# cucibala/FaceRecognizeOnnx

Measured on AMD Instinct MI355X. Metric: faces/sec end-to-end (detect+align+embed), batch=128 640x640, higher is better.
Workload: dtype f32; 1 GPU; C-headline: 128 frames 640x640 per GPU, SCRFD det_500m + decode + NMS, first 1 face(s)/frame aligned to 112x112, IResNet-50 (w600k_r50) embed, L2-norm; frames_per_gpu=128, faces_per_frame=1, weights=synthetic seeded (det seed 100, rec seed 200), input_residency=HBM-resident before the timed region, gallery_rows=0, topk=0, parallelism=frame-sharded x1, no data-path collective

## Files before the change

### facerecognizeonnx_amd/_lib.py

```python
from __future__ import annotations

import ctypes as C
import os
import subprocess

import numpy as np

_HERE = os.path.dirname(os.path.abspath(__file__))
LIB_PATH = os.path.join(_HERE, "libfacehip.so")
CSRC = os.path.join(_HERE, "csrc")

FACE_DTYPE = np.dtype([("x", "<i4"), ("y", "<i4"), ("w", "<i4"), ("h", "<i4"),
                       ("score", "<f4"), ("lm", "<f4", (10,))])
assert FACE_DTYPE.itemsize == 60


class FhFace(C.Structure):
    _fields_ = [("x", C.c_int32), ("y", C.c_int32), ("w", C.c_int32), ("h", C.c_int32),
                ("score", C.c_float), ("lm", C.c_float * 10)]


class FhFrame(C.Structure):
    _fields_ = [("bgr", C.c_void_p), ("rows", C.c_int32), ("cols", C.c_int32), ("step", C.c_int32)]

# ... 111 lines not shown
    "fh_tracker_get_state": (_i, [_vp, _i, _vp, _ip, _ip]),
    "fh_track_plan": (_i, [_vp, _i, _i, _vp, _vp]),
    "fh_track_update_dev": (_i, [_vp, _vp, _vp, _i, _i, _vp, _vp, _vp, _vp]),
    "fh_track_select_dev": (_i, [_vp, _vp, _i, _i, _vp, _vp, _vp, _vp, _vp, _vp]),
    "fh_pipeline_run_tracked_dev": (_i, [_vp, _vp, _vp, _vp, _i, _i, _i, _i, _ll, _vp, _f, _f, _i, _vp, _vp, _vp, _vp, _vp, _vp, _vp, _vp]),
    "fh_track_update_slots_dev": (_i, [_vp, _vp, _vp, _i, _i, _vp, _vp, _vp, _vp, _vp]),
    "fh_tracker_enable_identity": (_i, [_vp, _i, _i]),
    "fh_track_identify_dev": (_i, [_vp, _vp, _f, _vp, _vp, _vp, _vp, _i, _i, _i, _vp, _vp, _vp, _vp]),
    "fh_tracker_queries_dev": (_vp, [_vp]),
    "fh_tracker_get_identity": (_i, [_vp, _i, _vp, _vp]),
    "fh_pipeline_run_identified_dev": (_i, [_vp, _vp, _vp, _vp, _f, _vp, _i, _i, _i, _i, _ll, _vp, _f, _f, _i, _vp, _vp, _vp, _vp, _vp, _vp, _vp,
                                            _vp, _vp, _vp]),
    "fh_face_quality_dev": (_i, [_vp, _i, _i, _i, _i, _ll, _vp, _vp, _i, _vp, _vp]),
    "fh_face_quality_ragged_dev": (_i, [_vp, _i, _vp, _vp, _i, _vp, _vp]),
    "fh_tracker_set_bestshot": (_i, [_vp, _i, _i, _i, _i]),
    "fh_tracker_get_quality": (_i, [_vp, _i, _vp]),
    "fh_tracker_quality_dev": (_vp, [_vp]),
    "fh_track_update_q_dev": (_i, [_vp, _vp, _vp, _i, _i, _vp, _vp, _vp, _vp, _vp, _vp]),
    "fh_track_identify_q_dev": (_i, [_vp, _vp, _f, _vp, _vp, _vp, _vp, _vp, _i, _i, _i, _vp, _vp, _vp, _vp]),
    "fh_tracker_enable_relink": (_i, [_vp, _i, _f, _i]),
    "fh_track_identify_link_dev": (_i, [_vp, _vp, _f, _vp, _vp, _vp, _vp, _vp, _i, _i, _i, _vp, _vp, _vp, _vp, _vp]),
    "fh_tracker_get_links": (_i, [_vp, _i, _vp, _vp]),
    "fh_tracker_roots_dev": (_vp, [_vp]),
    "fh_gallery_create": (_vp, [_i]),
    "fh_gallery_destroy": (None, [_vp]),
    "fh_gallery_upload": (_i, [_vp, _vp, _ll, _i, _ll]),
    "fh_gallery_enroll": (_ll, [_vp, _vp, _ll, _i]),
    "fh_gallery_size": (_ll, [_vp]),
    "fh_gallery_label_dev": (_i, [_vp, _vp, _i, _f, _vp, _vp, _vp]),
    "fh_gallery_topk_dev": (_i, [_vp, _vp, _i, _i, _vp, _vp, _vp]),
    "fh_gallery_set_scan": (_i, [_vp, _i]),
    "fh_gallery_get_scan": (_i, [_vp]),
    "fh_gallery_scan_stats": (_i, [_vp, C.POINTER(_ll), C.POINTER(_ll)]),
    "fh_topk_merge_dev": (_i, [_vp, _vp, _i, _i, _i, _vp, _vp, _vp]),
    "fh_gallery_enroll_ids": (_ll, [_vp, _vp, _vp, _ll, _i]),
    "fh_gallery_upload_ids": (_i, [_vp, _vp, _vp, _ll, _i, _ll]),
    "fh_gallery_topk_ids_dev": (_i, [_vp, _vp, _i, _i, _vp, _vp, _vp, _vp]),
    "fh_gallery_label_ids_dev": (_i, [_vp, _vp, _i, _f, _vp, _vp, _vp]),
    "fh_gallery_remove_ids": (_ll, [_vp, _vp, _ll]),
    "fh_gallery_get_ids": (_ll, [_vp, _ll, _ll, _vp]),
    "fh_topk_merge_ids_dev": (_i, [_vp, _vp, _vp, _i, _i, _i, _vp, _vp, _vp, _vp]),
    "fh_gallery_group_ids": (_ll, [_vp, _ll, _vp, _vp, _vp]),
    "fh_gallery_fuse_ids": (_ll, [_vp, _vp, _i]),
    "fh_gallery_get_rows": (_ll, [_vp, _ll, _ll, _vp]),
    "fh_gallery_self_scores_dev": (_i, [_vp, _vp, _vp, _vp]),
    "fh_cluster_scores": (_i, [_vp, _i, _f, _i, _i, _vp, _vp]),
    "fh_gallery_cluster_dev": (_i, [_vp, _f, _i, _i, _vp, _vp, _vp]),
    "fh_hist_bin": (_i, [_f]),
    "fh_roc_from_hist": (_i, [_vp, _d, _vp]),
    "fh_gallery_pair_hist_dev": (_i, [_vp, _vp, _vp, _vp]),
    "fh_gallery_set_ids": (_ll, [_vp, _vp, _i]),
    "fh_gallery_set_tags": (_ll, [_vp, _ll, _ll, _vp, _i]),
    "fh_gallery_get_tags": (_ll, [_vp, _ll, _ll, _vp]),
    "fh_gallery_topk_tagged_dev": (_i, [_vp, _vp, _vp, _i, _i, _vp, _vp, _vp]),
    "fh_gallery_topk_ids_tagged_dev": (_i, [_vp, _vp, _vp, _i, _i, _vp, _vp, _vp, _vp]),
    "fh_gallery_label_tagged_dev": (_i, [_vp, _vp, _vp, _i, _f, _vp, _vp, _vp]),
    "fh_gallery_label_ids_tagged_dev": (_i, [_vp, _vp, _vp, _i, _f, _vp, _vp, _vp]),
    "fh_gallery_tag_stats": (_i, [_vp, C.POINTER(_ll), C.POINTER(_ll)]),
    "fh_tracker_set_stream_masks": (_i, [_vp, _vp]),
    "fh_gallery_range_dev": (_i, [_vp, _vp, _vp, _i, _f, _i, _vp, _vp, _vp, _vp, _vp]),
    "fh_range_from_scores": (_i, [_vp, _ll, _ll, _vp, C.c_uint32, _f, _i, C.POINTER(_ll), _vp, _vp]),
    "fh_comm_unique_id": (_i, [_vp]),
    "fh_comm_create": (_vp, [_i, _i, _vp, _i]),
    "fh_comm_destroy": (None, [_vp]),
    "fh_comm_rank": (_i, [_vp]),
    "fh_comm_world": (_i, [_vp]),
    "fh_comm_allgather_f32_dev": (_i, [_vp, _vp, _vp, _ll, _vp]),
    "fh_gallery_topk_sharded_dev": (_i, [_vp, _vp, _vp, _i, _i, _vp, _vp, _vp]),
    "fh_timing_enable": (_i, [_i]),
    "fh_timing_num_tags": (_i, []),
    "fh_timing_collect": (_i, [_vp, _vp, _vp, _vp, _i]),
    "fh_timing_collect_ops": (_i, [_vp, _vp, _vp, _i]),
    "fh_det_set_conv_cfg": (_i, [_vp, _i, _i]),
    "fh_rec_set_conv_cfg": (_i, [_vp, _i, _i]),
    "fh_memcpy_d2h": (_i, [_vp, _vp, C.c_size_t]),
    "fh_det_sync": (_i, [_vp, _vp]),
    "fh_rec_sync": (_i, [_vp, _vp]),
    "fh_imread": (_i, [C.c_char_p, C.POINTER(_vp), C.POINTER(_i), C.POINTER(_i)]),
    "fh_image_decode": (_i, [_vp, C.c_size_t, C.POINTER(_vp), C.POINTER(_i), C.POINTER(_i)]),
    "fh_image_free": (None, [_vp]),
    "fh_det_set_winograd": (_i, [_vp, _i]),
    "fh_rec_set_winograd": (_i, [_vp, _i]),
    "fh_rec_set_wino_fusion": (_i, [_vp, _i]),
    "fh_rec_set_shortcut_fold": (_i, [_vp, _i]),
    "fh_rec_set_precision": (_i, [_vp, _i, C.POINTER(C.c_float)]),
    "fh_rec_get_precision": (_i, [_vp]),
    "fh_det_set_cus": (_i, [_vp, _i]),
    "fh_rec_set_cus": (_i, [_vp, _i]),
    "fh_debug_streamk": (_i, [_i, _i]),
    "fh_debug_wino_slots": (_i, [_i]),
    "fh_debug_cluster_tiles": (_i, [_i]),
    "fh_debug_hist_copies": (_i, [_i]),
    "fh_debug_tag_skip": (_i, [_i]),
    "fh_debug_topk_merge_strided_dev": (_i, [_vp, _vp, _i, _i, _i, _ll, _vp, _vp, _vp]),
    "fh_set_graph_replay": (_i, [_i]),
    "fh_det_workspace_dev": (_vp, [_vp]),
    "fh_det_graph_stats": (_i, [_vp, _vp]),
    "fh_rec_graph_stats": (_i, [_vp, _vp]),
    "fh_det_set_fused_stem": (_i, [_vp, _i]),
    "fh_rec_set_fused_stem": (_i, [_vp, _i]),
    "fh_det_set_fused_front": (_i, [_vp, _i]),
    "fh_det_set_halo_conv": (_i, [_vp, _i]),
    "fh_resize_u8c3_dev": (_i, [_vp, _i, _i, _i, _vp, _i, _i, _i, _vp]),
    "fh_conv_forward_dev": (_i, [_vp, _vp, _vp, _vp, _i, _i, _i, _i, _i, _i, _i, _i, _i, _vp]),
    "fh_conv_winograd_dev": (_i, [_vp, _vp, _vp, _vp, _i, _i, _i, _i, _i, _vp]),
    "fh_conv_winograd_ex_dev": (_i, [_vp, _vp, _vp, _vp, _i, _i, _i, _i, _i, _i, _vp]),
    "fh_debug_pack_bf16x2_dev": (_i, [_vp, _vp, _ll]),
    "fh_debug_wino_gemm_rows": (_ll, [_i, _i, _i, _i, _i, _i]),
    "fh_debug_wino_gemm_dev": (_i, [_vp, _vp, _vp, _i, _i, _i, _i, _i, _i, _i, _vp]),
    "fh_debug_wino2_clock_mhz": (_d, []),
    "fh_conv_wino2_dev": (_i, [_vp, _vp, _vp, _vp, _vp, _vp, _i, _i, _i, _i, _i, _i, _i, _vp]),
    "fh_conv_wino2_ex_dev": (_i, [_vp, _vp, _vp, _vp, _vp, _vp, _vp, _vp, _vp, _i, _vp, _vp, _vp, _i, _i, _i, _i, _i, _i, _i, _vp]),
    "fh_conv_wt_rows": (_i, [_i]),
    "fh_conv_pack_weights": (_i, [_vp, _i, _i, _i, _vp]),
    "fh_conv_kpad": (_i, [_i]),
}

_LIB = None


def lib() -> C.CDLL:
    global _LIB
    if _LIB is None:
        path = build()
        path = os.environ.get("FACEHIP_LIB") or path
        try:
            import torch
        except ImportError:
            pass
        L = C.CDLL(path)
        for name, (res, args) in PROTOTYPES.items():
            fn = getattr(L, name)
            fn.restype = res
            fn.argtypes = args
        _LIB = L
    return _LIB


def last_error() -> str:
    return lib().fh_last_error().decode(errors="replace")


class FaceHipError(RuntimeError):
    pass


def check(rc: int, what: str) -> int:
    if rc < 0:
        raise FaceHipError(f"{what} failed ({rc}): {last_error()}")
    return rc
```

### facerecognizeonnx_amd/api.py

```python
from __future__ import annotations

import ctypes as C
from dataclasses import dataclass, field
from typing import List, Optional

import numpy as np

from . import _lib
from ._lib import FACE_DTYPE, TRACK_DTYPE, check


@dataclass
class FaceBox:
    box: tuple = (0, 0, 0, 0)
    score: float = 0.0
    landmarks: np.ndarray = field(default_factory=lambda: np.zeros((5, 2), np.float32))

    def to_record(self) -> np.ndarray:
        r = np.zeros(1, FACE_DTYPE)
        r[0]["x"], r[0]["y"], r[0]["w"], r[0]["h"] = self.box
        r[0]["score"] = self.score
        r[0]["lm"] = np.asarray(self.landmarks, np.float32).reshape(10)
        return r

# ... 140 lines not shown
            return np.zeros(0, FACE_DTYPE)
        t = self.tiling() if tiling is None else _tiling(tiling)
        if max_faces is None:
            views = check(_lib.lib().fh_tile_plan(a.shape[0], a.shape[1], C.byref(t), None, 0), "fh_tile_plan")
            max_faces = max(1, self.num_anchors() * views)
        out = np.zeros(max_faces, FACE_DTYPE)
        n = check(_lib.lib().fh_det_detect_tiled(self._h, a.ctypes.data, a.shape[0], a.shape[1], a.strides[0], C.byref(t),
                                                  scoreThreshold, nmsThreshold, out.ctypes.data, max_faces), "fh_det_detect_tiled")
        return out[:n].copy()

    def sync(self, stream: int = 0) -> None:
        check(_lib.lib().fh_det_sync(self._h, stream), "fh_det_sync")


class FaceRecognizer:
    def __init__(self):
        self._h = None

    def __del__(self):
        self.close()

    def close(self):
        if getattr(self, "_h", None) and _lib is not None and getattr(_lib, "_LIB", None) is not None:
            _lib._LIB.fh_rec_destroy(self._h)
        self._h = None

    def loadModel(self, modelPath: str) -> bool:
        self.close()
        self._h = _lib.lib().fh_rec_create(str(modelPath).encode())
        return bool(self._h)

    def extractFeature(self, image, face) -> np.ndarray:
        if not self._h:
            return np.zeros(0, np.float32)
        a = _img(image)
        if a is None:
            return np.zeros(0, np.float32)
        rec = face.to_record() if isinstance(face, FaceBox) else np.asarray(face, FACE_DTYPE).reshape(1)
        dim = self.feature_dim()
        out = np.zeros(dim, np.float32)
        n = check(_lib.lib().fh_rec_extract(self._h, a.ctypes.data, a.shape[0], a.shape[1], a.strides[0],
                                             rec.ctypes.data, out.ctypes.data, dim), "fh_rec_extract")
        return out[:n]

    def extractFeatureSimple(self, image) -> np.ndarray:
        if not self._h:
            return np.zeros(0, np.float32)
        a = _img(image)
        if a is None:
            return np.zeros(0, np.float32)
        dim = self.feature_dim()
        out = np.zeros(dim, np.float32)
        n = check(_lib.lib().fh_rec_extract_simple(self._h, a.ctypes.data, a.shape[0], a.shape[1], a.strides[0],
                                                    out.ctypes.data, dim), "fh_rec_extract_simple")
        return out[:n]

    @staticmethod
    def compareFaces(feature1, feature2) -> float:
        f1 = np.ascontiguousarray(feature1, np.float32).reshape(-1)
        f2 = np.ascontiguousarray(feature2, np.float32).reshape(-1)
        return float(_lib.lib().fh_compare(f1.ctypes.data, f1.size, f2.ctypes.data, f2.size))

    @property
    def handle(self):
        return self._h

    def feature_dim(self) -> int:
        return _lib.lib().fh_rec_feature_dim(self._h)

    def macs_per_face(self) -> float:
        return _lib.lib().fh_rec_macs_per_face(self._h)

    def set_chunk(self, n: int):
        check(_lib.lib().fh_rec_set_chunk(self._h, n), "fh_rec_set_chunk")

    def set_precision(self, mode: str = "fp32") -> float:
        import ctypes as C
        modes = {"fp32": 0, "bf16x2": 1}
        if mode not in modes:
            raise ValueError(f"precision {mode!r}: expected one of {sorted(modes)}")
        worst = C.c_float(0.0)
        check(_lib.lib().fh_rec_set_precision(self._h, modes[mode], C.byref(worst)), "fh_rec_set_precision")
        return float(worst.value)

    def precision(self) -> str:
        return "bf16x2" if _lib.lib().fh_rec_get_precision(self._h) == 1 else "fp32"

    def embed_aligned_dev(self, crops_ptr: int, n: int, out_ptr: int, raw_ptr: int = 0, stream: int = 0) -> int:
        return check(_lib.lib().fh_rec_embed_aligned_dev(self._h, crops_ptr, n, out_ptr, raw_ptr, stream),
                     "fh_rec_embed_aligned_dev")

    def sync(self, stream: int = 0) -> None:
        check(_lib.lib().fh_rec_sync(self._h, stream), "fh_rec_sync")


def pipeline_run_dev(det: FaceDetector, rec: FaceRecognizer, frames_ptr: int, n: int, rows: int, cols: int,
                     faces_per_frame: int, faces_ptr: int, frame_of_ptr: int, emb_ptr: int,
                     scoreThreshold: float = 0.5, nmsThreshold: float = 0.4, stream: int = 0) -> int:
    step = cols * 3
    return check(_lib.lib().fh_pipeline_run_dev(det.handle, rec.handle, frames_ptr, n, rows, cols, step, rows * step,
                                                scoreThreshold, nmsThreshold, faces_per_frame, faces_ptr,
                                                frame_of_ptr, emb_ptr, stream), "fh_pipeline_run_dev")


def pipeline_run_ragged_dev(det: FaceDetector, rec: FaceRecognizer, frames, faces_per_frame: int, faces_ptr: int, frame_of_ptr: int,
                            emb_ptr: int, scoreThreshold: float = 0.5, nmsThreshold: float = 0.4, stream: int = 0) -> int:
    arr = frame_array(frames)
    return check(_lib.lib().fh_pipeline_run_ragged_dev(det.handle, rec.handle, arr, _frame_count(arr), scoreThreshold, nmsThreshold,
                                                       faces_per_frame, faces_ptr, frame_of_ptr, emb_ptr, stream),
                 "fh_pipeline_run_ragged_dev")


def pipeline_run_tiled_dev(det: FaceDetector, rec: FaceRecognizer, frames, tiling, faces_per_frame: int, faces_ptr: int,
                           frame_of_ptr: int, emb_ptr: int, scoreThreshold: float = 0.5, nmsThreshold: float = 0.4,
                           stream: int = 0) -> int:
    arr, t = frame_array(frames), _tiling(tiling)
    return check(_lib.lib().fh_pipeline_run_tiled_dev(det.handle, rec.handle, arr, _frame_count(arr), C.byref(t), scoreThreshold,
                                                      nmsThreshold, faces_per_frame, faces_ptr, frame_of_ptr, emb_ptr, stream),
                 "fh_pipeline_run_tiled_dev")


def _stream_of(stream_of, n: int):
    if stream_of is None:
        return None, None
    a = np.ascontiguousarray(np.asarray(stream_of, np.int32).reshape(-1))
    if a.size != n:
        raise ValueError(f"stream_of holds {a.size} entries for {n} frames")
    return a, a.ctypes.data


def track_plan(stream_of, streams: int):
    a = np.ascontiguousarray(np.asarray(stream_of, np.int32).reshape(-1))
    order, starts = np.empty(max(a.size, 1), np.int32), np.empty(max(int(streams), 0) + 1, np.int32)
    check(_lib.lib().fh_track_plan(a.ctypes.data if a.size else None, a.size, int(streams), order.ctypes.data, starts.ctypes.data),
          "fh_track_plan")
    return order[:a.size].copy(), starts


def face_quality_dev(frames, det_ptr: int, counts_ptr: int, per_frame: int, quality_ptr: int, n: Optional[int] = None,
                     rows: Optional[int] = None, cols: Optional[int] = None, step: Optional[int] = None, stream: int = 0) -> int:
    if n is None:
        arr = frame_array(frames)
        return check(_lib.lib().fh_face_quality_ragged_dev(arr, _frame_count(arr), det_ptr, counts_ptr, per_frame, quality_ptr, stream),
                     "fh_face_quality_ragged_dev")
    step = cols * 3 if step is None else step
    return check(_lib.lib().fh_face_quality_dev(frames, n, rows, cols, step, rows * step, det_ptr, counts_ptr, per_frame, quality_ptr,
                                                stream), "fh_face_quality_dev")


class Tracker:

    def __init__(self, streams: int = 1, max_tracks: int = _lib.TRACK_MAX, iou_thr: float = 0.3, max_missed: int = 0, refresh: int = 0):
        self._h = _lib.lib().fh_tracker_create(int(streams), int(max_tracks), float(iou_thr), int(max_missed), int(refresh))
        if not self._h:
            raise _lib.FaceHipError(f"fh_tracker_create failed: {_lib.last_error()}")
        self.streams, self.max_tracks = int(streams), int(max_tracks)

    def close(self):
        if getattr(self, "_h", None):
            _lib.lib().fh_tracker_destroy(self._h)
            self._h = None

    def __del__(self):
        self.close()

    @property
# ... 496 lines not shown
```

### facerecognizeonnx_amd/csrc/api.cpp

```cpp
#include <algorithm>
#include <cmath>
#include <cstddef>
#include <cstdio>
#include <cstring>
#include <memory>
#include <string>
#include <vector>

#include "../../include/facehip.h"
#include "cluster_plan.h"
#include "range_plan.h"
#include "roc_plan.h"
#include "engine.h"
#include "group_ids.h"
#include "track_plan.h"

static_assert(sizeof(fh_face) == 60 && sizeof(fh::FaceRec) == 60, "FaceBox mirror must stay 60 bytes");
static_assert(sizeof(fh_frame) == 24 && sizeof(fh::FrameIn) == 24 && offsetof(fh_frame, rows) == offsetof(fh::FrameIn, rows) &&
              offsetof(fh_frame, step) == offsetof(fh::FrameIn, step), "fh_frame and the engine's FrameIn are one layout");
static_assert(sizeof(fh_track_state) == sizeof(fh::TrackState) && offsetof(fh_track_state, hits) == offsetof(fh::TrackState, hits) &&
              FH_TRACK_MAX == 64, "fh_track_state mirrors TrackState; one slot per lane of a wave");
static_assert(sizeof(fh_track_ident) == 16 && sizeof(fh::TrackIdent) == 16 && offsetof(fh_track_ident, score) == offsetof(fh::TrackIdent, score),
              "fh_track_ident mirrors TrackIdent");
static_assert(sizeof(fh_track_link) == 32 && sizeof(fh::TrackLink) == 32 && offsetof(fh_track_link, last_seen) == offsetof(fh::TrackLink, last_seen) &&
// ... 1361 lines not shown
static_assert(FH_HIST_BINS == fh::kHistBins && sizeof(fh_roc_point) == sizeof(fh::RocPoint) && sizeof(unsigned long long) == sizeof(uint64_t) &&
              offsetof(fh_roc_point, bin) == offsetof(fh::RocPoint, bin) && offsetof(fh_roc_point, impostor) == offsetof(fh::RocPoint, impostor),
              "fh_roc_point mirrors roc_plan.h");
int fh_hist_bin(float score) { return fh::hist_bin(score); }
int fh_roc_from_hist(const unsigned long long* hist, double max_far, fh_roc_point out[2]) {
    if (!hist || !out) return arg_error("fh_roc_from_hist: null argument");
    if (!(max_far >= 0.0 && max_far <= 1.0)) return arg_error("fh_roc_from_hist: need 0 <= max_far <= 1");
    fh::RocPoint pt[2];
    if (fh::roc_from_hist(reinterpret_cast<const uint64_t*>(hist), max_far, pt) < 0) {
        g_err = "fh_roc_from_hist: a plane of the histogram is empty (no genuine or no impostor pairs)";
        return FH_ERR_STATE;
    }
    for (int k = 0; k < 2; ++k)
        out[k] = fh_roc_point{pt[k].threshold, pt[k].bin, pt[k].true_accepts, pt[k].false_accepts, pt[k].genuine, pt[k].impostor};
    return FH_OK;
}
int fh_gallery_pair_hist_dev(fh_gallery* g, unsigned long long* d_hist, unsigned long long* d_nan, void* stream) {
    if (!g || !d_hist) return arg_error("fh_gallery_pair_hist_dev: null argument");
    if (g->g.size() > 0 && !g->g.labelled()) {
        g_err = "gallery: fh_gallery_pair_hist_dev needs a labelled gallery (rows enrolled with ids, or fh_gallery_set_ids)";
        return FH_ERR_STATE;
    }
    return guarded([&] { g->g.pair_hist_dev(d_hist, d_nan, S(stream)); return (int)FH_OK; });
}
int fh_debug_hist_copies(int copies) { fh::cluster_debug_hist_copies(copies); return 0; }

static_assert(FH_RANGE_MAX_CAP == fh::kRangeMaxCap && FH_TAG_ALL == fh::kRangeTagAll, "facehip.h mirrors range_plan.h");
int fh_range_from_scores(const float* scores, long long n, long long index_base, const uint32_t* tags, uint32_t mask, float threshold, int cap,
                         long long* count, float* out_scores, int* out_indices) {
    int listed = -1;
    const int rc = guarded([&] {
        listed = fh::range_from_scores(scores, n, index_base, tags, mask, threshold, cap, count, out_scores, out_indices);
        return 0;
    });
    if (rc < 0) return rc;
    return listed < 0 ? arg_error("fh_range_from_scores: bad argument (null scores or count, NaN threshold, cap outside 1..1024, index beyond 31 bits)")
                      : listed;
}
int fh_gallery_range_dev(fh_gallery* g, const float* d_queries, const uint32_t* d_masks, int nq, float threshold, int cap, long long* d_counts,
                         float* d_scores, int* d_indices, int* d_ids, void* stream) {
    if (!g) return arg_error("fh_gallery_range_dev: null handle");
    if (nq < 0 || nq > 256) return arg_error("fh_gallery_range_dev: need 0 <= nq <= 256");
    if (cap < 1 || cap > FH_RANGE_MAX_CAP) return arg_error("fh_gallery_range_dev: need 1 <= cap <= FH_RANGE_MAX_CAP");
    if (threshold != threshold) return arg_error("fh_gallery_range_dev: the threshold is a NaN");
    if (g->g.dim() % 64) return arg_error("fh_gallery_range_dev: the gallery's dim must be a multiple of 64");
    if (nq == 0) return 0;
    if (!d_queries || !d_counts) return arg_error("fh_gallery_range_dev: null argument");
    if (d_ids && g->g.size() > 0 && !g->g.labelled()) {
        g_err = "gallery: fh_gallery_range_dev with d_ids needs a labelled gallery (rows enrolled with ids, or fh_gallery_set_ids)";
        return FH_ERR_STATE;
    }
    return guarded([&] { g->g.range_dev(d_queries, d_masks, nq, threshold, cap, d_counts, d_scores, d_indices, d_ids, S(stream)); return nq; });
}

int fh_debug_topk_merge_strided_dev(const float* ps, const int* pi, int nparts, int nq, int k, long long part_stride, float* scores, int* indices,
                                    void* stream) {
    if (!ps || !pi || !scores || !indices) return arg_error("fh_debug_topk_merge_strided_dev: null argument");
    if (nparts <= 0 || nq <= 0 || k <= 0 || k > 16 || (long)nparts * k > 65536 || part_stride < (long long)nq * k)
        return arg_error("fh_debug_topk_merge_strided_dev: bad size");
    return guarded([&] {
        fh::launch_topk_merge_strided(ps, pi, nparts, nq, k, (long)part_stride, scores, indices, S(stream));
        FH_HIP(hipGetLastError());
        return nq;
    });
}

int fh_timing_enable(int on) { fh::KernelTimer::get().enabled = on != 0; return FH_OK; }
int fh_timing_num_tags(void) { return fh::KernelTimer::kTags; }
int fh_timing_collect(double* ms, double* flops, double* bytes, long long* launches, int n) {
    if (!ms || !flops || !bytes || !launches || n < fh::KernelTimer::kTags) return arg_error("fh_timing_collect: need fh_timing_num_tags()-entry arrays");
    return guarded([&] { fh::KernelTimer::get().collect(ms, flops, bytes, launches); return fh::KernelTimer::kTags; });
}
int fh_timing_collect_ops(double* ms, double* flops, int* tag, int cap) {
    if (!ms || !flops || !tag || cap <= 0) return arg_error("fh_timing_collect_ops: bad argument");
    return guarded([&] { return fh::KernelTimer::get().collect_ops(ms, flops, tag, cap); });
}
int fh_det_set_conv_cfg(fh_det* d, int cfg, int stream_k) {
    if (!d) return arg_error("null handle");
    d->det.net().force_cfg = cfg; d->det.net().sk_enable = stream_k != 0;
    return FH_OK;
}
int fh_det_set_winograd(fh_det* d, int on) { if (!d) return arg_error("null handle"); d->det.net().winograd = on != 0; return FH_OK; }
int fh_rec_set_winograd(fh_rec* r, int on) { if (!r) return arg_error("null handle"); r->rec.net().winograd = on != 0; return FH_OK; }
int fh_rec_set_wino_fusion(fh_rec* r, int on) { if (!r) return arg_error("null handle"); r->rec.net().fuse_wino = on != 0; return FH_OK; }
int fh_rec_set_precision(fh_rec* r, int mode, float* worst_out) {
    if (!r || (mode != FH_PREC_FP32 && mode != FH_PREC_BF16X2)) return arg_error("fh_rec_set_precision: bad argument");
    if (worst_out) *worst_out = 0.f;
    Owns owns(&r->rec.net());
    if (mode == FH_PREC_FP32) return guarded([&] { r->rec.net().set_bf16x2(false, nullptr); return (int)FH_OK; });
    return guarded([&] {
        fh::Net& net = r->rec.net();
        const int n = 64, dim = r->rec.dim();
        const size_t crop = (size_t)net.in_h() * net.in_w() * 3;
        std::vector<uint8_t> h((size_t)n * crop);
        uint32_t st = 0x9E3779B9u;
        for (int i = 0; i < n; ++i) {
            const int amp = 16 + 3 * i;
            for (size_t e = 0; e < crop; ++e) {
                st = st * 1664525u + 1013904223u;
                const int px = (int)(e / 3) % net.in_w(), py = (int)(e / 3) / net.in_w();
                const int v = 128 + ((px * (i + 1) + py * (n - i)) % 97 - 48) + (int)((st >> 24) % (2 * amp + 1)) - amp;
                h[(size_t)i * crop + e] = (uint8_t)std::min(255, std::max(0, v));
            }
        }
        fh::DevBuf dc, de;
        dc.ensure(h.size()); de.ensure((size_t)2 * n * dim * sizeof(float));
        FH_HIP(hipMemcpy(dc.p, h.data(), h.size(), hipMemcpyHostToDevice));
        const bool was = net.bf16x2();
        net.set_bf16x2(false, nullptr);
        r->rec.embed_aligned_dev(dc.as<uint8_t>(), n, de.as<float>(), nullptr);
        const int layers = net.set_bf16x2(true, nullptr);
        if (layers == 0) { net.set_bf16x2(was, nullptr); throw std::runtime_error("fh_rec_set_precision: this model has no layer with a split-bf16 form"); }
        struct Rollback { fh::Net& n; bool armed = true; ~Rollback() { if (armed) { try { n.set_bf16x2(false, nullptr); } catch (...) {} } } } rollback{net};
        r->rec.embed_aligned_dev(dc.as<uint8_t>(), n, de.as<float>() + (size_t)n * dim, nullptr);
        std::vector<float> e((size_t)2 * n * dim);
        FH_HIP(hipDeviceSynchronize());
        FH_HIP(hipMemcpy(e.data(), de.p, e.size() * sizeof(float), hipMemcpyDeviceToHost));
        double worst = 0;
        for (int i = 0; i < n; ++i) {
            double dot = 0, na = 0, nb = 0;
            for (int c = 0; c < dim; ++c) {
                const double a = e[(size_t)i * dim + c], b = e[(size_t)(n + i) * dim + c];
                dot += a * b; na += a * a; nb += b * b;
            }
            const double err = (na > 0 && nb > 0) ? 1.0 - dot / std::sqrt(na * nb) : 1.0;
            worst = std::max(worst, std::isfinite(err) ? err : 1.0);
        }
        if (worst_out) *worst_out = (float)worst;
        double gate = 1e-3;
        if (const char* g = getenv("FACEHIP_PRECISION_GATE")) gate = std::min(gate, atof(g));
        if (!(worst < gate))
            throw std::runtime_error("fh_rec_set_precision: split-bf16 embeddings differ from fp32 by 1 - cos = " + std::to_string(worst) +
                                 " (gate " + std::to_string(gate) + "): staying fp32");
        rollback.armed = false;
        return layers;
    });
}
int fh_rec_get_precision(fh_rec* r) { return r && r->rec.net().bf16x2() ? FH_PREC_BF16X2 : FH_PREC_FP32; }
int fh_rec_set_shortcut_fold(fh_rec* r, int on) { if (!r) return arg_error("null handle"); r->rec.net().fold_shortcut = on != 0; return FH_OK; }
int fh_det_set_halo_conv(fh_det* d, int on) { if (!d) return arg_error("null handle"); d->det.net().halo_conv = on != 0; return FH_OK; }
int fh_det_set_cus(fh_det* d, int cus) { if (!d || cus < 0) return arg_error("bad argument"); d->det.net().cus = cus; return FH_OK; }
int fh_rec_set_cus(fh_rec* r, int cus) { if (!r || cus < 0) return arg_error("bad argument"); r->rec.net().cus = cus; return FH_OK; }
int fh_det_set_fused_stem(fh_det* d, int on) { if (!d) return arg_error("null handle"); d->det.net().fuse_stem = on != 0; return FH_OK; }
int fh_det_set_fused_front(fh_det* d, int on) { if (!d) return arg_error("null handle"); d->det.net().fuse_front = on != 0; return FH_OK; }
int fh_rec_set_fused_stem(fh_rec* r, int on) { if (!r) return arg_error("null handle"); r->rec.net().fuse_stem = on != 0; return FH_OK; }
int fh_rec_set_conv_cfg(fh_rec* r, int cfg, int stream_k) {
    if (!r) return arg_error("null handle");
    r->rec.net().force_cfg = cfg; r->rec.net().sk_enable = stream_k != 0;
    return FH_OK;
}

int fh_memcpy_d2h(void* dst, const void* src, size_t bytes) {
    if (!dst || !src) return arg_error("fh_memcpy_d2h: null argument");
    return guarded([&] { FH_HIP(hipDeviceSynchronize()); FH_HIP(hipMemcpy(dst, src, bytes, hipMemcpyDeviceToHost)); return 0; });
}
int fh_resize_u8c3_dev(const uint8_t* src, int sh, int sw, int sstep, uint8_t* dst, int dh, int dw, int dstep, void* stream) {
    if (!src || !dst || sh <= 0 || sw <= 0 || dh <= 0 || dw <= 0) return arg_error("fh_resize_u8c3_dev: bad argument");
    return guarded([&] {
        fh::launch_resize_u8c3(src, (long)sh * sstep, sh, sw, sstep, dst, (long)dh * dstep, dh, dw, dstep, 1, S(stream));
        FH_HIP(hipGetLastError());
        return 0;
    });
}
int fh_conv_winograd_ex_dev(const float* d_in, const float* w_ohwi, const float* d_bias, float* d_out, int batch, int h, int w, int cin,
                            int cout, int precision, void* stream) {
    if (!d_in || !w_ohwi || !d_out || cin % 32 || cout % 4 || (precision != FH_PREC_FP32 && precision != FH_PREC_BF16X2))
        return arg_error("fh_conv_winograd_dev: bad argument");
    const bool bf2 = precision == FH_PREC_BF16X2;
    Owns owns(nullptr);
    return guarded([&] {
        if (bf2 && !fh::wino_gemm_ok_bf16x2(cin, cout)) throw std::runtime_error("winograd: this layer has no split-bf16 GEMM");
        const int rows = fh::conv_wt_rows(cout);
        std::vector<float> u36((size_t)36 * rows * cin, 0.f), uf((size_t)cout * cin);
        std::vector<double> uall((size_t)cout * cin * 36);
        for (int co = 0; co < cout; ++co)
            for (int ci = 0; ci < cin; ++ci) {
                double g[9];
                for (int t = 0; t < 9; ++t) g[t] = w_ohwi[((size_t)co * 9 + t) * cin + ci];
                fh::wino_filter_transform(g, &uall[((size_t)co * cin + ci) * 36]);
            }
        for (int f = 0; f < 36; ++f) {
            for (size_t e = 0; e < uf.size(); ++e) uf[e] = (float)uall[e * 36 + f];
            fh::conv_pack_weights(uf.data(), cout, cin, 1, u36.data() + (size_t)f * rows * cin);
        }
        const size_t tiles = (size_t)batch * ((h + 3) / 4) * ((w + 3) / 4);
        fh::DevBuf dU, dV, dM;
        dU.ensure(u36.size() * sizeof(float));
        dV.ensure((36 * (size_t)fh::wino_rows((long)tiles) + 100 * 128) * cin * sizeof(float));
        dM.ensure((36 * (size_t)fh::wino_rows((long)tiles) + 100 * 128) * cout * sizeof(float));
        FH_HIP(hipMemcpy(dU.p, u36.data(), u36.size() * sizeof(float), hipMemcpyHostToDevice));
        fh::DevBuf dUp;
        if (bf2) {
            dUp.ensure(u36.size() * sizeof(float));
            fh::launch_pack_bf16x2(dU.as<float>(), dUp.as<float>(), (long)u36.size(), S(stream));
        }
        static fh::DevBuf slabs;
        static unsigned slabs_gen = 0;
        if (!slabs.p) { slabs.ensure(fh::conv_slab_floats() * sizeof(float)); fh::conv_workspace_init(slabs.as<float>()); slabs_gen = fh::conv_error_generation(); }
        if (slabs_gen != fh::conv_error_generation()) { fh::conv_workspace_reset_async(slabs.as<float>(), S(stream)); slabs_gen = fh::conv_error_generation(); }
        fh::ConvArgs a{};
        a.in = d_in; a.bias = d_bias; a.out1 = d_out; a.slabs = slabs.as<float>(); a.sk_enable = 1;
        a.B = batch; a.H = h; a.W = w; a.Ho = h; a.Wo = w; a.Cin = cin; a.Cout = cout; a.ks = 3; a.stride = 1; a.pad = 1;
        a.act = (int)fh::Act::NONE; a.res_mode = (int)fh::ResMode::NONE;
        fh::launch_conv_winograd(a, (bf2 ? dUp : dU).as<float>(), dV.as<float>(), dM.as<float>(), 2, nullptr, nullptr, S(stream), bf2);
        FH_HIP(hipStreamSynchronize(S(stream)));
        return 0;
    });
}
int fh_conv_winograd_dev(const float* d_in, const float* w_ohwi, const float* d_bias, float* d_out, int batch, int h, int w, int cin,
                         int cout, void* stream) {
    return fh_conv_winograd_ex_dev(d_in, w_ohwi, d_bias, d_out, batch, h, w, cin, cout, FH_PREC_FP32, stream);
}
int fh_debug_pack_bf16x2_dev(const float* d_in, float* d_out, long long n) {
    if (!d_in || !d_out || n < 0 || n % 4) return arg_error("fh_debug_pack_bf16x2_dev: bad argument (n % 4 == 0)");
    return guarded([&] {
        fh::launch_pack_bf16x2(d_in, d_out, (long)n, nullptr);
        FH_HIP(hipGetLastError());
        FH_HIP(hipStreamSynchronize(nullptr));
        return 0;
    });
}
static long long wino_gemm_rows(int batch, int h, int w, int k, int n, int mixed, fh::WinoPlanes* pl) {
    if (batch <= 0 || h <= 0 || w <= 0 || k <= 0 || n <= 0 || k % 32 || n % 32) return -1;
    if (!mixed) return 36LL * fh::wino_rows((long)batch * ((h + 3) / 4) * ((w + 3) / 4));
    fh::WinoPlanes p{};
    if (!fh::wino_mix_layout(batch, h, w, k, n, &p)) return -2;
    if (pl) *pl = p;
    return 128LL * p.total_tiles;
}
long long fh_debug_wino_gemm_rows(int batch, int h, int w, int k, int n, int mixed) {
    const long long r = wino_gemm_rows(batch, h, w, k, n, mixed, nullptr);
    if (r == -2) return arg_error("fh_debug_wino_gemm_rows: the mixed tiling does not apply to this layer");
    if (r < 0) return arg_error("fh_debug_wino_gemm_rows: bad argument (k % 32 == 0, n % 32 == 0)");
    return r;
}
int fh_debug_wino_gemm_dev(const float* d_V, const float* d_U, float* d_M, int batch, int h, int w, int k, int n, int precision, int mixed,
                           void* stream) {
    if (!d_V || !d_U || !d_M || (precision != FH_PREC_FP32 && precision != FH_PREC_BF16X2))
        return arg_error("fh_debug_wino_gemm_dev: bad argument");
    fh::WinoPlanes pl{};
    const long long rows = wino_gemm_rows(batch, h, w, k, n, mixed, &pl);
    if (rows == -2) return arg_error("fh_debug_wino_gemm_dev: the mixed tiling does not apply to this layer");
    if (rows < 0) return arg_error("fh_debug_wino_gemm_dev: bad argument (k % 32 == 0, n % 32 == 0)");
    const bool bf2 = precision == FH_PREC_BF16X2;
    Owns owns(nullptr);
    return guarded([&] {
        if (bf2 && !fh::wino_gemm_ok_bf16x2(k, n)) throw std::runtime_error("winograd: this layer has no split-bf16 GEMM");
        const size_t nv = (size_t)rows * k, nu = (size_t)36 * fh::conv_wt_rows(n) * k;
        fh::DevBuf dVp, dUp;
        if (bf2) {
            dVp.ensure(nv * sizeof(float)); dUp.ensure(nu * sizeof(float));
            fh::launch_pack_bf16x2(d_V, dVp.as<float>(), (long)nv, S(stream));
            fh::launch_pack_bf16x2(d_U, dUp.as<float>(), (long)nu, S(stream));
        }
        fh::ConvArgs a{};
        a.B = batch; a.H = h; a.W = w; a.Ho = h; a.Wo = w; a.Cin = k; a.Cout = n; a.ks = 3; a.stride = 1; a.pad = 1;
        a.act = (int)fh::Act::NONE; a.res_mode = (int)fh::ResMode::NONE;
        fh::launch_wino_gemm(a, bf2 ? dUp.as<float>() : d_U, bf2 ? dVp.as<float>() : d_V, d_M, 2, bf2, S(stream), mixed ? &pl : nullptr);
        FH_HIP(hipGetLastError());
        FH_HIP(hipStreamSynchronize(S(stream)));
        return 0;
    });
}
int fh_conv_wino2_ex_dev(const float* d_in, const float* w_ohwi, const float* d_bias, const float* d_slope, const float* d_res, float* d_out,
                         float* d_out2, const float* d_s2, const float* d_t2, int n_outs, float* const* d_outs, const int* oc0, const int* oact,
                         int batch, int h, int w, int cin, int cout, int act, int bias_cls, void* stream) {
    if (!d_in || !w_ohwi || batch <= 0 || h <= 0 || w <= 0 || cin != 64 || cout <= 0) return arg_error("fh_conv_wino2_dev: bad argument (cin = 64, positive sizes)");
    if (n_outs < 0 || n_outs > 3 || (n_outs > 0 && (!d_outs || !oc0 || !oact))) return arg_error("fh_conv_wino2_dev: bad merged-output description");
    if (n_outs == 0 && ((!d_out && !d_out2) || cout % 64)) return arg_error("fh_conv_wino2_dev: plain layers need an output and cout % 64 == 0");
    if (d_out2 && (!d_s2 || !d_t2)) return arg_error("fh_conv_wino2_dev: a second output needs its scale and shift");
    Owns owns(nullptr);
    return guarded([&] {
        fh::ConvArgs a{};
        a.in = d_in; a.bias = d_bias; a.slope = d_slope; a.res = d_res; a.out1 = d_out; a.out2 = d_out2; a.s2 = d_s2; a.t2 = d_t2;
        a.B = batch; a.H = h; a.W = w; a.Ho = h; a.Wo = w; a.Cin = cin; a.Cout = cout; a.ks = 3; a.stride = 1; a.pad = 1;
        a.act = act; a.bias_cls = bias_cls; a.res_mode = d_res ? (int)fh::ResMode::SAME : (int)fh::ResMode::NONE;
        a.n_outs = n_outs;
        for (int g = 0; g < n_outs; ++g) { a.outs[g] = d_outs[g]; a.oact[g] = oact[g]; a.oc0[g] = oc0[g]; }
        if (n_outs > 0) a.oc0[n_outs] = oc0[n_outs];
        if (!fh::wino2_ok(a)) throw std::runtime_error("fh_conv_wino2_dev: layer shape not supported by the fused F(2x2) kernel");
        std::vector<float> u(fh::wino2_weight_floats(cin, cout));
        fh::wino2_pack_weights(w_ohwi, cout, cin, u.data());
        fh::DevBuf dU;
        dU.ensure(u.size() * sizeof(float));
        FH_HIP(hipMemcpy(dU.p, u.data(), u.size() * sizeof(float), hipMemcpyHostToDevice));
        a.wt = dU.as<float>();
        fh::launch_wino2(a, S(stream));
        FH_HIP(hipGetLastError());
        FH_HIP(hipStreamSynchronize(S(stream)));
        return 0;
    });
}
int fh_conv_wino2_dev(const float* d_in, const float* w_ohwi, const float* d_bias, const float* d_slope, const float* d_res, float* d_out,
                      int batch, int h, int w, int cin, int cout, int act, int bias_cls, void* stream) {
    return fh_conv_wino2_ex_dev(d_in, w_ohwi, d_bias, d_slope, d_res, d_out, nullptr, nullptr, nullptr, 0, nullptr, nullptr, nullptr, batch, h, w,
                                cin, cout, act, bias_cls, stream);
}
double fh_debug_wino2_clock_mhz(void) { return fh::wino2_debug_clock_mhz(); }
int fh_conv_wt_rows(int cout) { return fh::conv_wt_rows(cout); }
int fh_conv_pack_weights(const float* w_ohwi, int cout, int cin, int ksize, float* dst_packed) {
    if (!w_ohwi || !dst_packed || cout <= 0 || cin <= 0) return arg_error("fh_conv_pack_weights: bad argument");
    memset(dst_packed, 0, (size_t)fh::conv_wt_rows(cout) * fh::conv_kpad(ksize * ksize * cin) * sizeof(float));
    fh::conv_pack_weights(w_ohwi, cout, cin, ksize, dst_packed);
    return 0;
}
int fh_conv_kpad(int ktot) { return fh::conv_kpad(ktot); }
const float* fh_det_workspace_dev(fh_det* d) { return d ? d->det.net().workspace() : nullptr; }
int fh_set_graph_replay(int on) { g_graph_replay = on != 0; return FH_OK; }
int fh_det_graph_stats(fh_det* d, long long* replays) {
    if (!d) return arg_error("null handle");
    if (replays) *replays = d->gcall.replays;
    return (int)d->gcall.nodes;
}
int fh_rec_graph_stats(fh_rec* r, long long* replays) {
    if (!r) return arg_error("null handle");
    if (replays) *replays = r->gcall.replays + r->gcall_simple.replays;
    return (int)(r->gcall.nodes ? r->gcall.nodes : r->gcall_simple.nodes);
}
int fh_debug_wino_slots(int slots) { fh::wino_debug_slots(slots); return 0; }
int fh_debug_streamk(int drop_publish, int timeout_ms) { fh::conv_debug_streamk(drop_publish, timeout_ms); return 0; }
int fh_conv_forward_dev(const float* in, const float* wt, const float* bias, float* out, int batch, int h, int w, int cin, int cout,
                        int ks, int stride, int kpad, int cfg, void* stream) {
    if (!in || !wt || !out || batch <= 0 || (ks != 1 && ks != 3) || cin % 4) return arg_error("fh_conv_forward_dev: bad argument");
    Owns owns(nullptr);
    return guarded([&] {
        fh::ConvArgs a{};
        const int pad = ks / 2;
        a.in = in; a.wt = wt; a.bias = bias; a.out1 = out;
        a.B = batch; a.H = h; a.W = w; a.Cin = cin; a.Cout = cout; a.ks = ks; a.stride = stride; a.pad = pad;
        a.Ho = (h + 2 * pad - ks) / stride + 1; a.Wo = (w + 2 * pad - ks) / stride + 1;
        a.Kpad = kpad;
        static fh::DevBuf slabs;
        static unsigned slabs_gen = 0;
        if (!slabs.p) { slabs.ensure(fh::conv_slab_floats() * sizeof(float)); fh::conv_workspace_init(slabs.as<float>()); slabs_gen = fh::conv_error_generation(); }
        if (slabs_gen != fh::conv_error_generation()) { fh::conv_workspace_reset_async(slabs.as<float>(), S(stream)); slabs_gen = fh::conv_error_generation(); }
        a.slabs = slabs.as<float>(); a.sk_enable = 1;
        fh::launch_conv(a, cfg, S(stream));
        FH_HIP(hipGetLastError());
        return 0;
    });
}
// ... 7 lines not shown
```

### facerecognizeonnx_amd/csrc/engine.cpp

```cpp
#include "engine.h"

#include "group_ids.h"
#include "roc_plan.h"
#include "track_plan.h"

#include <atomic>
#include <climits>
#include <cstdio>
#include <cstdlib>
#include <algorithm>
#include <cmath>
#include <cstring>

namespace fh {

void hip_check(hipError_t e, const char* what) {
    if (e != hipSuccess) throw std::runtime_error(std::string("HIP error: ") + hipGetErrorString(e) + " in " + what);
}

static std::atomic<unsigned long long> g_layout_epoch{1};
unsigned long long layout_epoch() { return g_layout_epoch.load(std::memory_order_relaxed); }

DevBuf::~DevBuf() {
    if (p) { (void)hipFree(p); g_layout_epoch.fetch_add(1, std::memory_order_relaxed); }
// ... 95 lines not shown
        for (int co = 0; co < c.Cout; ++co) {
            double tap_shift[9];
            for (int t = 0; t < 9; ++t) {
                double acc = 0;
                for (int ci = 0; ci < c.Cin; ++ci) acc += (double)c.weight[((size_t)co * 9 + t) * c.Cin + ci] * pr.t2[ci];
                tap_shift[t] = acc;
            }
            for (int ry = 0; ry < 3; ++ry)
                for (int rx = 0; rx < 3; ++rx) {
                    double b = c.bias[co];
                    for (int ky = 0; ky < 3; ++ky)
                        for (int kx = 0; kx < 3; ++kx) {
                            const bool in_y = !(ry == 0 && ky == 0) && !(ry == 2 && ky == 2);
                            const bool in_x = !(rx == 0 && kx == 0) && !(rx == 2 && kx == 2);
                            if (in_y && in_x) b += tap_shift[ky * 3 + kx];
                        }
                    b9[(size_t)(ry * 3 + rx) * c.Cout + co] = (float)b;
                }
            for (int t = 0; t < 9; ++t)
                for (int ci = 0; ci < c.Cin; ++ci) c.weight[((size_t)co * 9 + t) * c.Cin + ci] *= pr.s2[ci];
        }
        c.bias = b9;
        dev_[i].bn_fold_src = c.bn_src;
        dev_[c.bn_src].bn_fold_dst = true;
    }
    for (size_t i = 0; i < plan_.ops.size(); ++i) {
        const POp& op = plan_.ops[i];
        DevOp& d = dev_[i];
        if (op.kind == OpKind::DWPW) {
            d.dww = push(op.dw_weight.data(), op.dw_weight.size());
            d.dwb = push(op.dw_bias.data(), op.dw_bias.size());
        }
        if (op.kind == OpKind::CONV || op.kind == OpKind::GEMM || op.kind == OpKind::DWPW) {
            const int Ktot = op.ks * op.ks * op.Cin;
            d.Kpad = conv_kpad(Ktot);
            const int rows = conv_wt_rows(op.Cout);
            std::vector<float> packed((size_t)rows * d.Kpad, 0.f);
            conv_pack_weights(op.weight.data(), op.Cout, op.Cin, op.ks, packed.data());
            d.wt = push(packed.data(), packed.size());
            if (op.kind == OpKind::CONV) {
                ConvArgs probe{};
                probe.ks = op.ks; probe.stride = op.stride; probe.pad = op.pad; probe.Cin = op.Cin; probe.Cout = op.Cout; probe.act = (int)op.act;
                probe.res_mode = (int)op.res_mode; probe.H = op.H; probe.W = op.W;
                float dummy = 0.f;
                probe.out2 = op.out2 >= 0 ? &dummy : nullptr;
                probe.bias_cls = dev_[i].bn_fold_src >= 0 ? 1 : 0;
                if (conv_halo_ok(probe) && op.Ho * op.Wo >= 400) {
                    std::vector<float> wf(conv_halo_wfrag_floats(op.Cin, op.Cout));
                    conv_halo_pack_weights(op.weight.data(), op.Cout, op.Cin, wf.data());
                    d.wfrag = push(wf.data(), wf.size());
                    d.halo = true;
                }
            }
            if (op.kind == OpKind::CONV && op.Cin < kWinoMinCin) {
                ConvArgs probe{};
                probe.ks = op.ks; probe.stride = op.stride; probe.pad = op.pad; probe.Cin = op.Cin; probe.Cout = op.Cout; probe.act = (int)op.act;
                probe.res_mode = (int)op.res_mode; probe.H = op.H; probe.W = op.W; probe.Ho = op.Ho; probe.Wo = op.Wo;
                probe.n_outs = (int)op.outs.size(); probe.bias_cls = dev_[i].bn_fold_src >= 0 ? 1 : 0;
                float dummy2 = 0.f;
                probe.out2 = op.out2 >= 0 ? &dummy2 : nullptr;
                if (wino2_ok(probe)) {
                    std::vector<float> u(wino2_weight_floats(op.Cin, op.Cout));
                    wino2_pack_weights(op.weight.data(), op.Cout, op.Cin, u.data());
                    d.w2 = push(u.data(), u.size());
                    d.w2ok = true;
                }
            }
            if (op.kind == OpKind::CONV && op.ks == 3 && op.stride == 1 && op.pad == 1 && op.Cin >= kWinoMinCin && op.Cin % 32 == 0 &&
                op.Cout % 4 == 0 && op.outs.empty() && op.res_mode != ResMode::UP2X) {
                std::vector<float> u36((size_t)36 * rows * op.Cin, 0.f), uf((size_t)op.Cout * op.Cin);
                std::vector<double> uall((size_t)op.Cout * op.Cin * 36);
                for (int co = 0; co < op.Cout; ++co)
                    for (int ci = 0; ci < op.Cin; ++ci) {
                        double g[9];
                        for (int t = 0; t < 9; ++t) g[t] = op.weight[((size_t)co * 9 + t) * op.Cin + ci];
                        wino_filter_transform(g, &uall[((size_t)co * op.Cin + ci) * 36]);
                    }
                for (int f = 0; f < 36; ++f) {
                    for (size_t e = 0; e < uf.size(); ++e) uf[e] = (float)uall[e * 36 + f];
                    conv_pack_weights(uf.data(), op.Cout, op.Cin, 1, u36.data() + (size_t)f * rows * op.Cin);
                }
                d.w36 = push(u36.data(), u36.size());
                d.w36n = u36.size();
                d.wino = true;
                d.bf2 = wino_gemm_ok_bf16x2(op.Cin, op.Cout);
                const size_t tiles = (size_t)((op.H + 3) / 4) * ((op.W + 3) / 4);
                wino_elems_ = std::max(wino_elems_, 36 * tiles * (size_t)std::max(op.Cin, op.Cout));
                wino_maxc_ = std::max(wino_maxc_, (size_t)std::max(op.Cin, op.Cout));
            }
        } else if (op.kind == OpKind::DWCONV || op.kind == OpKind::DWGLOBAL || op.kind == OpKind::GCONV) {
            d.wt = push(op.weight.data(), op.weight.size());
        }
        if (!op.bias.empty()) d.bias = push(op.bias.data(), op.bias.size());
        if (!op.slope.empty()) { d.slope = push(op.slope.data(), op.slope.size()); d.has_slope = true; }
        if (!op.s2.empty()) { d.s2 = push(op.s2.data(), op.s2.size()); d.t2 = push(op.t2.data(), op.t2.size()); d.has_aff = true; }
    }
    for (size_t i = 0; i < plan_.ops.size(); ++i) {
        const POp& c = plan_.ops[i];
        if (c.sc_src < 0 || dev_[i].bn_fold_src >= 0 || c.bias.size() != (size_t)c.Cout) continue;
        if (dev_[i].wino || dev_[i].halo) continue;
        const POp& x = plan_.ops[c.sc_src];
        const int K9 = 9 * c.Cin, K = K9 + x.Cin, rows = conv_wt_rows(c.Cout);
        std::vector<float> w((size_t)rows * K, 0.f), b((size_t)c.Cout);
        for (int co = 0; co < c.Cout; ++co) {
            std::copy_n(&c.weight[(size_t)co * K9], K9, &w[(size_t)co * K]);
            std::copy_n(&x.weight[(size_t)co * x.Cin], x.Cin, &w[(size_t)co * K + K9]);
            b[co] = c.bias[co] + (x.bias.empty() ? 0.f : x.bias[co]);
        }
        dev_[i].wt_sc = push(w.data(), w.size());
        dev_[i].bias_sc = push(b.data(), b.size());
        dev_[i].Kpad_sc = K;
        dev_[i].sc_src = c.sc_src;
        dev_[c.sc_src].sc_dst = true;
    }
    for (size_t i = 0; i < plan_.ops.size(); ++i) {
        const int prod = plan_.ops[i].bn_src;
        if (!dev_[i].wino || prod <= 0 || !dev_[prod].has_aff) continue;
        dev_[i].aff_src = prod; dev_[prod].aff_dst = (int)i;
    }
    for (size_t i = 0; i + 1 < plan_.ops.size(); ++i) {
        const POp& a = plan_.ops[i];
        const POp& b = plan_.ops[i + 1];
        if (!dev_[i].wino || !dev_[i + 1].wino || a.H != b.H || a.W != b.W || a.Cout != b.Cin || !wino_can_fuse(a.H, a.W, a.Cout, false)) continue;
        int feed = -1;
        if (dev_[i + 1].aff_src == (int)i) feed = 1;
        else if (a.out >= 0 && b.in == a.out) feed = 0;
        else if (a.out2 >= 0 && b.in == a.out2) feed = 1;
        if (feed < 0) continue;
        int other_uses = 0;
        if (a.out >= 0) {
            for (const POp& o : plan_.ops)
                for (int x : {o.in, o.in2, o.res}) if (x == a.out) ++other_uses;
            for (const auto& o : plan_.outputs) if (o.tensor == a.out) ++other_uses;
            if (b.in == a.out) --other_uses;
        }
        const bool writes_out2 = a.out2 >= 0 && dev_[i + 1].aff_src != (int)i;
        if (!wino_can_fuse(a.H, a.W, a.Cout, other_uses > 0 || a.res >= 0 || writes_out2)) continue;
        dev_[i].fuse_next = true; dev_[i].fuse_feed_aff = feed == 1; dev_[i].fuse_keep_out1 = other_uses > 0;
    }
    {
        const POp& op = plan_.ops[0];
        stem_ok_ = op.kind == OpKind::CONV && op.in == plan_.input && op.ks == 3 && op.Cin == 4 && op.res < 0 && op.outs.empty() &&
                   op.Cout % 4 == 0 && op.Cout <= 64 && (op.stride == 1 || op.stride == 2);
        if (stem_ok_) {
            std::vector<float> w27((size_t)27 * op.Cout);
            for (int co = 0; co < op.Cout; ++co)
                for (int t = 0; t < 9; ++t)
                    for (int ci = 0; ci < 3; ++ci) w27[(size_t)(t * 3 + ci) * op.Cout + co] = op.weight[((size_t)co * 9 + t) * 4 + ci];
            dev_[0].w27 = push(w27.data(), w27.size());
            std::vector<float> wf((size_t)27 * op.Cout), bf((size_t)op.Cout);
            for (int co = 0; co < op.Cout; ++co) {
                double sum = 0;
                for (int t = 0; t < 9; ++t)
                    for (int j = 0; j < 3; ++j) {
                        const float w = op.weight[((size_t)co * 9 + t) * 4 + (2 - j)];
                        wf[(size_t)(t * 3 + j) * op.Cout + co] = w / 128.0f;
                        sum += w;
                    }
                bf[co] = (float)((double)op.bias[co] - 127.5 / 128.0 * sum);
            }
            dev_[0].wf = push(wf.data(), wf.size());
            dev_[0].bf = push(bf.data(), bf.size());
            if (op.Cout % 16 == 0) {
                std::vector<unsigned> fr((size_t)(op.Cout / 16) * 3 * 64 * 4, 0u);
                stem_pack_wfrag(wf.data(), op.Cout, fr.data());
                std::vector<float> asf(fr.size());
// ... 24 lines not shown
    (void)hipDeviceSynchronize();
    if (device >= 0 && device != cur && cur >= 0) (void)hipSetDevice(cur);
    conv_error_record_release(p);
}

void Net::reserve(int max_batch) {
    if (max_batch <= cap_) return;
    cap_ = max_batch;
    arena_.ensure(plan_.arena_elems * (size_t)cap_ * sizeof(float));
    if (partial_.bytes < conv_slab_floats() * sizeof(float)) {
        partial_.ensure(conv_slab_floats() * sizeof(float));
        conv_workspace_init(partial_.as<float>());
        if (!sk_rec_.p) { sk_rec_.p = conv_error_record_new(); (void)hipGetDevice(&sk_rec_.device); }
        if (!sk_rec_.p) throw std::runtime_error("HIP error: cannot allocate the stream-K watchdog record");
        sk_gen_ = conv_error_generation();
    }
    if (wino_elems_) {
        const size_t pad = 36 * 256 * wino_maxc_;
        wino_v_.ensure((wino_elems_ * (size_t)cap_ + pad) * sizeof(float));
        wino_m_.ensure((wino_elems_ * (size_t)cap_ + pad) * sizeof(float));
    }
    FH_HIP(hipMemset(arena_.p, 0, arena_.bytes));
}

void Net::run_u8(const uint8_t* src, long img_stride, int srcH, int srcW, int step, int batch, hipStream_t s) {
    if (batch <= 0) return;
    if (batch > cap_) throw std::runtime_error("Net::run_u8: batch exceeds reserved capacity");
    if (stem_ok_ && fuse_stem && front_ok_ && fuse_front && srcW >= 2) {
        const POp& st = plan_.ops[0];
        const POp& op = plan_.ops[1];
        const DevOp& d0 = dev_[0];
        const DevOp& d = dev_[1];
        const float* P = params_.as<float>();
        ConvArgs a{};
        a.wt = P + d.wt; a.bias = P + d.bias;
        a.out1 = tensor_ptr(op.out);
        a.dw_w = P + d.dww; a.dw_b = P + d.dwb; a.dw_act = (int)op.dw_act; a.dw_stride = op.dw_stride;
        a.B = batch; a.H = op.H; a.W = op.W; a.Cin = op.Cin; a.Ho = op.Ho; a.Wo = op.Wo; a.Cout = op.Cout;
        a.ks = 1; a.stride = 1; a.pad = 0; a.Kpad = d.Kpad; a.act = (int)op.act;
        a.u8_src = src; a.u8_img_stride = img_stride; a.u8_step = step; a.u8_srcH = srcH; a.u8_srcW = srcW; a.u8_inH = plan_.inH; a.u8_inW = plan_.inW;
        a.slabs = partial_.as<float>();
        a.u8_stride = st.stride; a.stem_act = (int)st.act; a.stem_wf = P + d0.wf; a.stem_bf = P + d0.bf;
        a.stem_wfrag = reinterpret_cast<const unsigned*>(P + d0.wfr);
        a.cus = cus;
        a.t_flops = 2.0 * (st.macs + op.macs) * batch;
        a.t_bytes = ((double)srcH * srcW * 3 + (double)op.Ho * op.Wo * op.Cout * 4) * batch;
        launch_dwpw(a, s);
        run(batch, s, 2);
        return;
    }
    if (stem_ok_ && fuse_stem) {
        const POp& op = plan_.ops[0];
        const DevOp& d = dev_[0];
        const float* P = params_.as<float>();
        KernelTimer& timer = KernelTimer::get();
        timer.begin(s);
        StemArgs a{};
        a.src = src; a.img_stride = img_stride; a.srcH = srcH; a.srcW = srcW; a.step = step; a.B = batch; a.inH = plan_.inH; a.inW = plan_.inW;
        a.stride = op.stride; a.Cout = op.Cout; a.w27 = P + d.w27; a.bias = P + d.bias; a.wf = P + d.wf; a.biasf = P + d.bf;
        a.wfrag = d.wfr ? reinterpret_cast<const unsigned*>(P + d.wfr) : nullptr;
        a.slope = d.has_slope ? P + d.slope : nullptr; a.act = (int)op.act; a.cus = cus;
        a.out1 = op.out >= 0 ? tensor_ptr(op.out) : nullptr; a.out2 = op.out2 >= 0 && !d.bn_fold_dst ? tensor_ptr(op.out2) : nullptr;
        if (d.has_aff) { a.s2 = P + d.s2; a.t2 = P + d.t2; }
        launch_stem(a, s);
        timer.end(s, 5, 2.0 * op.macs * batch, op.bytes * batch);
        run(batch, s, 1);
        return;
    }
    launch_det_preprocess(src, img_stride, srcH, srcW, step, batch, plan_.inH, plan_.inW, srcH, srcW, input(), s);
    run(batch, s, 0);
}

int Net::set_bf16x2(bool on, hipStream_t s) {
    int layers = 0;
    size_t total = 0;
    for (auto& d : dev_) if (d.wino && d.bf2) { d.w36p = total; total += d.w36n; ++layers; }
    if (on && layers > 0 && w36_bf_.bytes < total * sizeof(float)) {
        w36_bf_.ensure(total * sizeof(float));
        for (const auto& d : dev_)
            if (d.wino && d.bf2) launch_pack_bf16x2(params_.as<float>() + d.w36, w36_bf_.as<float>() + d.w36p, (long)d.w36n, s);
        FH_HIP(hipStreamSynchronize(s));
    }
    bf16x2_ = on && layers > 0;
    return on ? layers : 0;
}

void Net::run(int batch, hipStream_t s, int first_op) {
    if (batch <= 0) return;
    if ((sk_gen_ != conv_error_generation() || conv_error_pending(sk_rec_.p)) && partial_.p) {
        conv_workspace_reset_async(partial_.as<float>(), s);
        sk_gen_ = conv_error_generation();
    }
    if (batch > cap_) throw std::runtime_error("Net::run: batch exceeds reserved capacity");
    const float* P = params_.as<float>();
    KernelTimer& timer = KernelTimer::get();
    bool v_ready = false;
    for (size_t i = (size_t)first_op; i < plan_.ops.size(); ++i) {
        const POp& op = plan_.ops[i];
        const DevOp& d = dev_[i];
        int tag = 5;
        const bool dense = op.kind == OpKind::CONV || op.kind == OpKind::GEMM || op.kind == OpKind::DWPW;
        if (!dense) timer.begin(s);
        switch (op.kind) {
            case OpKind::CONV:
            case OpKind::GEMM: {
                if (d.sc_dst && fold_shortcut && force_cfg < 0) break;
                ConvArgs a{};
                a.in = tensor_ptr(op.in);
                a.wt = P + d.wt;
                a.bias = P + d.bias;
                a.slope = d.has_slope ? P + d.slope : nullptr;
                a.res = op.res >= 0 ? tensor_ptr(op.res) : nullptr;
                a.out1 = op.out >= 0 ? tensor_ptr(op.out) : nullptr;
                a.out2 = op.out2 >= 0 ? tensor_ptr(op.out2) : nullptr;
                if (d.bn_fold_dst) a.out2 = nullptr;
                if (d.bn_fold_src >= 0) { a.in = tensor_ptr(plan_.ops[d.bn_fold_src].out); a.bias_cls = 1; }
                if (d.aff_dst >= 0 && winograd) {
                    const POp& c = plan_.ops[d.aff_dst];
                    if ((long)batch * ((c.H + 3) / 4) * ((c.W + 3) / 4) >= kWinoMinTiles) a.out2 = nullptr;
                }
                a.s2 = d.has_aff ? P + d.s2 : nullptr;
                a.t2 = d.has_aff ? P + d.t2 : nullptr;
                a.slabs = partial_.as<float>();
                a.sk_err = sk_rec_.p;
                a.sk_enable = sk_enable ? 1 : 0;
                a.cus = cus;
                a.no_pw = force_cfg >= 0 ? 1 : 0;
                a.B = batch; a.H = op.H; a.W = op.W; a.Cin = op.Cin; a.Ho = op.Ho; a.Wo = op.Wo; a.Cout = op.Cout;
                a.ks = op.ks; a.stride = op.stride; a.pad = op.pad; a.Kpad = d.Kpad;
                a.act = (int)op.act; a.res_mode = (int)op.res_mode;
                a.n_outs = (int)op.outs.size();
                for (int g = 0; g < a.n_outs && g < 3; ++g) { a.outs[g] = tensor_ptr(op.outs[g]); a.oact[g] = op.out_act[g]; a.oc0[g] = op.out_c0[g]; }
                if (a.n_outs > 0) a.oc0[a.n_outs] = op.out_c0[a.n_outs];
                const long M = (long)batch * op.Ho * op.Wo;
                int cfg = force_cfg >= 0 ? force_cfg : conv_pick_cfg(M, op.Cout);
                if (force_cfg < 0 && cfg == 0 && ((M + 127) / 128) * ((op.Cout + 127) / 128) < 128) cfg = 3;
                a.t_flops = 2.0 * op.macs * batch; a.t_bytes = op.bytes * batch;
                if (d.sc_src >= 0 && fold_shortcut && force_cfg < 0) {
                    const POp& x = plan_.ops[d.sc_src];
                    a.wt = P + d.wt_sc; a.bias = P + d.bias_sc; a.Kpad = d.Kpad_sc;
                    a.res = nullptr; a.res_mode = (int)ResMode::NONE;
                    a.sc_in = tensor_ptr(x.in); a.sc_H = x.H; a.sc_W = x.W; a.sc_C = x.Cin; a.sc_stride = x.stride;
                    a.t_flops += 2.0 * x.macs * batch;
                }
                if (d.halo && halo_conv && force_cfg < 0) {
                    launch_conv_halo(a, P + d.wfrag, s);
                    tag = 9;
                    break;
                }
                if (d.w2ok && winograd && force_cfg < 0 && d.sc_src < 0 && wino2_blocks(a) >= wino2_min_blocks()) {
                    a.wt = P + d.w2;
                    launch_wino2(a, s);
                    break;
                }
                const bool use_wino = d.wino && winograd && (long)batch * ((op.H + 3) / 4) * ((op.W + 3) / 4) >= kWinoMinTiles;
                if (use_wino) {
                    const int wcfg = force_cfg >= 0 ? force_cfg : 2;
                    const bool bf2 = bf16x2_ && d.bf2 && force_cfg < 0;
                    WinoPlanes pl;
                    const bool mix = wcfg == 2 && wino_mix_layout(batch, op.H, op.W, op.Cin, op.Cout, &pl);
                    if (!v_ready) {
                        const float* in_s = nullptr; const float* in_t = nullptr;
                        if (d.aff_src >= 0) {
                            a.in = tensor_ptr(plan_.ops[d.aff_src].out);
                            in_s = P + dev_[d.aff_src].s2; in_t = P + dev_[d.aff_src].t2;
                        }
                        if (mix) launch_wino_mix(a, pl, nullptr, wino_v_.as<float>(), 0, in_s, in_t, bf2, s);
                        else launch_wino_input(a, wino_v_.as<float>(), in_s, in_t, bf2, s);
                    }
                    launch_wino_gemm(a, bf2 ? w36_bf_.as<float>() + d.w36p : P + d.w36, wino_v_.as<float>(), wino_m_.as<float>(), wcfg, bf2, s,
                                     mix ? &pl : nullptr);
                    v_ready = false;
                    if (d.fuse_next && fuse_wino && i + 1 < plan_.ops.size()) {
                        const POp& nx = plan_.ops[i + 1];
                        const bool next_wino = dev_[i + 1].wino && (long)batch * ((nx.H + 3) / 4) * ((nx.W + 3) / 4) >= kWinoMinTiles;
                        const bool next_mix = next_wino && wcfg == 2 && wino_mix_layout(batch, nx.H, nx.W, nx.Cin, nx.Cout, nullptr);
                        if (next_wino && mix == next_mix) {
                            ConvArgs e = a;
                            if (!d.fuse_keep_out1) e.out1 = nullptr;
                            const bool pack_next = bf16x2_ && dev_[i + 1].bf2 && force_cfg < 0;
                            if (mix) launch_wino_mix(e, pl, wino_m_.as<float>(), wino_v_.as<float>(), d.fuse_feed_aff ? 1 : 0, nullptr, nullptr, pack_next, s);
                            else launch_wino_fused(e, wino_m_.as<float>(), wino_v_.as<float>(), d.fuse_feed_aff ? 1 : 0, pack_next, s);
                            v_ready = true;
                        }
                    }
                    if (!v_ready) {
                        if (mix) launch_wino_mix(a, pl, wino_m_.as<float>(), nullptr, 0, nullptr, nullptr, false, s);
                        else launch_wino_output(a, wino_m_.as<float>(), s);
                    }
                    tag = 7;
                    break;
                }
                launch_conv(a, cfg, s);
                tag = cfg;
                break;
            }
            case OpKind::DWPW: {
                ConvArgs a{};
                a.in = tensor_ptr(op.in);
                a.wt = P + d.wt; a.bias = P + d.bias;
                a.out1 = tensor_ptr(op.out);
                a.dw_w = P + d.dww; a.dw_b = P + d.dwb; a.dw_act = (int)op.dw_act; a.dw_stride = op.dw_stride;
                a.B = batch; a.H = op.H; a.W = op.W; a.Cin = op.Cin; a.Ho = op.Ho; a.Wo = op.Wo; a.Cout = op.Cout;
                a.ks = 1; a.stride = 1; a.pad = 0; a.Kpad = d.Kpad; a.act = (int)op.act;
                a.t_flops = 2.0 * op.macs * batch; a.t_bytes = op.bytes * batch;
                a.slabs = partial_.as<float>();
                a.cus = cus;
                launch_dwpw(a, s);
                break;
            }
            case OpKind::DWCONV:
                launch_dwconv3x3(tensor_ptr(op.in), P + d.wt, P + d.bias, tensor_ptr(op.out), batch, op.H, op.W, op.Cin, op.stride,
                                 (int)op.act, d.has_slope ? P + d.slope : nullptr, s);
                tag = 4;
                break;
            case OpKind::DWGLOBAL:
                launch_dwglobal(tensor_ptr(op.in), P + d.wt, P + d.bias, tensor_ptr(op.out), batch, op.ks * op.ks, op.Cin, (int)op.act,
                                d.has_slope ? P + d.slope : nullptr, s);
                break;
            case OpKind::GCONV:
                launch_gconv3x3(tensor_ptr(op.in), P + d.wt, P + d.bias, tensor_ptr(op.out), batch, op.H, op.W, op.Cin,
                                (int)(op.weight_group), op.stride, (int)op.act, d.has_slope ? P + d.slope : nullptr, s);
                tag = 4;
                break;
            case OpKind::AFFINE:
                launch_affine(tensor_ptr(op.in), P + d.s2, P + d.t2, tensor_ptr(op.out), (long)batch * op.H * op.W, op.Cin, s);
                break;
            case OpKind::ACT:
                launch_act(tensor_ptr(op.in), d.has_slope ? P + d.slope : nullptr, tensor_ptr(op.out), (long)batch * op.H * op.W,
                           op.Cin, (int)op.act, s);
                break;
            case OpKind::ADD:
                launch_add(tensor_ptr(op.in), tensor_ptr(op.in2), tensor_ptr(op.out), (long)batch * op.H * op.W * op.Cin, s);
                break;
            case OpKind::UPSAMPLE:
                launch_upsample2x(tensor_ptr(op.in), tensor_ptr(op.out), batch, op.H, op.W, op.Cin, s);
                break;
        }
        if (!dense) timer.end(s, tag, 2.0 * op.macs * batch, op.bytes * batch);
        if (debug_sync()) {
            fprintf(stderr, "[facehip] op %zu %s batch %d done-launch\n", i, op.name.c_str(), batch); fflush(stderr);
            const hipError_t e1 = hipGetLastError(), e2 = hipStreamSynchronize(s);
            if (e1 != hipSuccess || e2 != hipSuccess)
                throw std::runtime_error("HIP error after op " + std::to_string(i) + " (" + op.name + "): " + hipGetErrorString(e1 != hipSuccess ? e1 : e2));
        }
    }
    FH_HIP(hipGetLastError());
}

Detector::Detector(const std::string& onnx_path) : net_(onnx_path, 640, 640) {
    const auto& outs = net_.plan().outputs;
    const int H = net_.in_h(), W = net_.in_w();
    if (outs.size() == 9) {
        static const int cols[9] = {1, 1, 1, 4, 4, 4, 10, 10, 10};
// ... 173 lines not shown
}

void TileTable::upload(const TilePlan& p, hipStream_t s) {
    const size_t vb = p.views.size() * sizeof(ViewDesc), sb = p.segs.size() * sizeof(FrameSeg);
    char* h = static_cast<char*>(st_.stage(vb + sb));
    if (vb) memcpy(h, p.views.data(), vb);
    if (sb) memcpy(h + vb, p.segs.data(), sb);
    V_ = (int)p.views.size();
    st_.send(vb + sb, s);
}

void postprocess_views(PostArgs a, int n_frames, const TileTable* tab, float nms_thr, int* sup, FaceRec* out, int max_out, int* counts,
                       hipStream_t s) {
    FH_HIP(hipMemsetAsync(a.count, 0, (size_t)n_frames * sizeof(int), s));
    a.views = tab ? tab->views() : nullptr;
    a.segs = tab ? tab->segs() : nullptr;
    if (a.rows) launch_rows_threshold(a, s);
    else launch_scrfd_decode(a, s);
    launch_sort_nms(a.cand, a.keys, a.count, a.segs, a.cap, n_frames, nms_thr, out, counts, max_out, sup, s);
    FH_HIP(hipGetLastError());
}

PostArgs Detector::post_source(int V, float score_thr) {
    PostArgs a{};
    if (predecoded_) { a.rows = net_.output(0); a.n_rows = anchors_; a.feat = feat_; }
    else {
        for (int i = 0; i < 3; ++i) { a.score[i] = net_.output(i); a.bbox[i] = net_.output(3 + i); a.kps[i] = net_.output(6 + i); }
        a.inH = net_.in_h(); a.inW = net_.in_w();
    }
    a.V = V; a.cap = cap_; a.border = -1; a.thr = score_thr;
    a.cand = cand_.as<FaceRec>(); a.keys = keys_.as<unsigned long long>(); a.count = count_.as<int>();
    return a;
}

int Detector::run_network_tiled_dev(const FrameIn* frames, int n, const Tiling& t, hipStream_t s) {
    const int V = tplan_.plan(frames, n, t, net_.in_w(), net_.in_h(), cap_, kTileMaxViews);
    if (V < 0) throw std::invalid_argument("tiled detection: more than FH_TILE_MAX_VIEWS views in one call, split the batch");
    frames_table_.upload(frames, n, 0, 0, s);
    ttab_.upload(tplan_, s);
    if (V > 0) run_network_ragged_dev(tplan_.view_frames.data(), V, s);
    return V;
}

void Detector::detect_tiled_dev(const FrameIn* frames, int n, const Tiling& t, float score_thr, float nms_thr, FaceRec* out, int max_out,
                                int* counts, hipStream_t s) {
    if (n <= 0) return;
    const int V = run_network_tiled_dev(frames, n, t, s);
    if (V == 0 || anchors_ <= 0) { FH_HIP(hipMemsetAsync(counts, 0, (size_t)n * sizeof(int), s)); return; }
    keys_.ensure(tplan_.key_total * sizeof(unsigned long long));
    ws_.ensure(tplan_.key_total * sizeof(int));
    count_.ensure((size_t)n * sizeof(int));
    PostArgs a = post_source(V, score_thr);
    a.border = t.border;
    postprocess_views(a, n, &ttab_, nms_thr, ws_.as<int>(), out, max_out, counts, s);
}

void Detector::run_input_dev(const float* input, int n, hipStream_t s) {
    reserve(n, 0, 0);
    ragged_ = false;
    const size_t per = (size_t)net_.in_h() * net_.in_w() * 4;
    FH_HIP(hipMemcpyAsync(net_.input(), input, (size_t)n * per * sizeof(float), hipMemcpyDeviceToDevice, s));
    net_.run(n, s);
}

void Detector::postprocess_dev(int n, float score_thr, float nms_thr, FaceRec* out, int max_out, int* counts, hipStream_t s) {
    if (anchors_ <= 0) { FH_HIP(hipMemsetAsync(counts, 0, (size_t)n * sizeof(int), s)); return; }
    if (ragged_ && n > table_.size()) throw std::runtime_error("detector: more frames than the last ragged call described");
    PostArgs a = post_source(n, score_thr);
    a.scale = scale_;
    a.scales = ragged_ ? table_.scales() : nullptr;
    postprocess_views(a, n, nullptr, nms_thr, ws_.as<int>(), out, max_out, counts, s);
}

void Detector::detect_dev(const uint8_t* frames, int n, int rows, int cols, int step, long stride, float score_thr, float nms_thr,
                          FaceRec* out, int max_out, int* counts, hipStream_t s) {
    if (n <= 0) return;
    run_network_dev(frames, n, rows, cols, step, stride, s);
    postprocess_dev(n, score_thr, nms_thr, out, max_out, counts, s);
}

Recognizer::Recognizer(const std::string& onnx_path) : net_(onnx_path, 112, 112) {
    const auto& o = net_.plan().outputs.at(0);
    dim_ = o.rows * o.cols;
}

void Recognizer::embed_aligned_dev(const uint8_t* crops, int n, float* out, hipStream_t s, float* raw_out) {
    const int H = net_.in_h(), W = net_.in_w();
    net_.reserve(std::min(n, max_chunk));
    for (int off = 0; off < n; off += max_chunk) {
        const int c = std::min(max_chunk, n - off);
        net_.run_u8(crops + (size_t)off * H * W * 3, (long)H * W * 3, H, W, W * 3, c, s);
        if (raw_out) FH_HIP(hipMemcpyAsync(raw_out + (size_t)off * dim_, net_.output(0), (size_t)c * dim_ * sizeof(float), hipMemcpyDeviceToDevice, s));
        launch_l2_normalize(net_.output(0), out + (size_t)off * dim_, c, dim_, s);
    }
    FH_HIP(hipGetLastError());
}

void Recognizer::embed_input_dev(const float* input, int n, float* out, hipStream_t s, float* raw_out) {
    const size_t per = (size_t)net_.in_h() * net_.in_w() * 4;
    net_.reserve(std::min(n, max_chunk));
    for (int off = 0; off < n; off += max_chunk) {
        const int c = std::min(max_chunk, n - off);
        FH_HIP(hipMemcpyAsync(net_.input(), input + (size_t)off * per, (size_t)c * per * sizeof(float), hipMemcpyDeviceToDevice, s));
        net_.run(c, s);
        if (raw_out) FH_HIP(hipMemcpyAsync(raw_out + (size_t)off * dim_, net_.output(0), (size_t)c * dim_ * sizeof(float), hipMemcpyDeviceToDevice, s));
        launch_l2_normalize(net_.output(0), out + (size_t)off * dim_, c, dim_, s);
    }
    FH_HIP(hipGetLastError());
}

void Recognizer::align_dev(const uint8_t* frames, int rows, int cols, int step, long stride, const FaceRec* faces,
                           const int* frame_of, int n, uint8_t* crops, int* ok, hipStream_t s) {
    launch_align(frames, stride, rows, cols, step, faces, frame_of, n, net_.in_h(), net_.in_w(), crops, ok, s);
    FH_HIP(hipGetLastError());
}

void Recognizer::embed_faces_dev(const uint8_t* frames, int rows, int cols, int step, long stride, const FaceRec* faces,
                                 const int* frame_of, int n, float* out, int* ok, hipStream_t s) {
    if (n <= 0) return;
    const size_t crop = (size_t)net_.in_h() * net_.in_w() * 3;
    crops_.ensure((size_t)n * crop);
    ok_.ensure((size_t)n * sizeof(int));
    int* okp = ok ? ok : ok_.as<int>();
    align_dev(frames, rows, cols, step, stride, faces, frame_of, n, crops_.as<uint8_t>(), okp, s);
    embed_aligned_dev(crops_.as<uint8_t>(), n, out, s);
}

void Recognizer::align_table_dev(const FrameDesc* table, int n_frames, const FaceRec* faces, const int* frame_of, int n, uint8_t* crops,
                                 int* ok, hipStream_t s) {
    launch_align_ragged(table, n_frames, faces, frame_of, n, net_.in_h(), net_.in_w(), crops, ok, s);
    FH_HIP(hipGetLastError());
}

void Recognizer::embed_faces_table_dev(const FrameDesc* table, int n_frames, const FaceRec* faces, const int* frame_of, int n, float* out,
                                       int* ok, hipStream_t s) {
    if (n <= 0) return;
    const size_t crop = (size_t)net_.in_h() * net_.in_w() * 3;
    crops_.ensure((size_t)n * crop);
    ok_.ensure((size_t)n * sizeof(int));
    align_table_dev(table, n_frames, faces, frame_of, n, crops_.as<uint8_t>(), ok ? ok : ok_.as<int>(), s);
    embed_aligned_dev(crops_.as<uint8_t>(), n, out, s);
}

void Recognizer::align_ragged_dev(const FrameIn* frames, int n_frames, const FaceRec* faces, const int* frame_of, int n, uint8_t* crops,
                                  int* ok, hipStream_t s) {
    align_table_dev(table_.upload(frames, n_frames, 0, 0, s), n_frames, faces, frame_of, n, crops, ok, s);
}

void Recognizer::embed_faces_ragged_dev(const FrameIn* frames, int n_frames, const FaceRec* faces, const int* frame_of, int n, float* out,
                                        int* ok, hipStream_t s) {
    if (n <= 0) return;
    embed_faces_table_dev(table_.upload(frames, n_frames, 0, 0, s), n_frames, faces, frame_of, n, out, ok, s);
}

void Recognizer::resize_embed_dev(const uint8_t* frames, int n, int rows, int cols, int step, long stride, float* out, hipStream_t s) {
    const int H = net_.in_h(), W = net_.in_w();
    crops_.ensure((size_t)n * H * W * 3);
    launch_resize_u8c3(frames, stride, rows, cols, step, crops_.as<uint8_t>(), (long)H * W * 3, H, W, W * 3, n, s);
    embed_aligned_dev(crops_.as<uint8_t>(), n, out, s);
}

Tracker::Tracker(int streams, int max_tracks, float iou_thr, int max_missed, int refresh)
    : streams_(streams), p_{max_tracks, iou_thr, max_missed, refresh, 1, 1, 1} {
    state_.ensure((size_t)streams * (2 * sizeof(int) + (size_t)max_tracks * sizeof(TrackState)));
    reset(-1);
}
// ... 189 lines not shown
```

### facerecognizeonnx_amd/csrc/engine.h

```cpp
#pragma once
#include <hip/hip_runtime.h>

#include <cstdint>
#include <stdexcept>
#include <string>
#include <utility>
#include <vector>

#include "kernels.h"
#include "plan.h"
#include "tile_plan.h"

namespace fh {


struct DevBuf {
    void* p = nullptr;
    size_t bytes = 0;
    DevBuf() = default;
    DevBuf(const DevBuf&) = delete;
    DevBuf& operator=(const DevBuf&) = delete;
    ~DevBuf();
    void ensure(size_t n);
    void swap(DevBuf& o) { std::swap(p, o.p); std::swap(bytes, o.bytes); }
    void grow(size_t n, size_t keep) {
        if (n <= bytes) return;
        if (keep == 0) return ensure(n);
        DevBuf bigger;
        bigger.ensure(n);
        FH_HIP(hipMemcpy(bigger.p, p, keep, hipMemcpyDeviceToDevice));
        swap(bigger);
    }
    template <class T> T* as() const { return reinterpret_cast<T*>(p); }
};

unsigned long long layout_epoch();

class Net {
  public:
    Net(const std::string& onnx_path, int default_h, int default_w);
    void reserve(int max_batch);
    float* input() const { return arena_.as<float>() + plan_.tensors[plan_.input].offset * (size_t)cap_; }
    float* output(int i) const { return tensor_ptr(plan_.outputs[i].tensor); }
    void run(int batch, hipStream_t s, int first_op = 0);
    void run_u8(const uint8_t* src, long img_stride, int srcH, int srcW, int step, int batch, hipStream_t s);
    bool fuse_stem = true;
    bool fuse_front = true;
    const Plan& plan() const { return plan_; }
    int in_h() const { return plan_.inH; }
    int in_w() const { return plan_.inW; }
    int capacity() const { return cap_; }
    bool winograd = true;
    bool halo_conv = true;
    bool fold_shortcut = true;
    bool fuse_wino = true;
    int set_bf16x2(bool on, hipStream_t s);
    bool bf16x2() const { return bf16x2_; }
    int cus = 0;
    int force_cfg = -1;
    bool sk_enable = true;
    long long config_word() const {
        return (long long)fuse_stem | (long long)fuse_front << 1 | (long long)winograd << 2 | (long long)halo_conv << 3 |
               (long long)fold_shortcut << 4 | (long long)fuse_wino << 5 | (long long)bf16x2_ << 6 | (long long)sk_enable << 7 |
               (long long)(cus & 0xffff) << 8 | (long long)((force_cfg + 1) & 0xff) << 24;
    }

  private:
    struct DevOp {
        size_t wt = 0, bias = 0, slope = 0, s2 = 0, t2 = 0;
        bool has_slope = false, has_aff = false;
        size_t w27 = 0;
        size_t wfr = 0;
        size_t wf = 0, bf = 0;
        size_t dww = 0, dwb = 0;
        size_t w36 = 0;
        size_t w36n = 0, w36p = 0;
        bool bf2 = false;
        size_t wfrag = 0;
        bool halo = false;
        bool wino = false;
        size_t w2 = 0;
        bool w2ok = false;
        int aff_src = -1;
        int aff_dst = -1;
        int bn_fold_src = -1;
        bool bn_fold_dst = false;
        int sc_src = -1;
        size_t wt_sc = 0, bias_sc = 0;
        int Kpad_sc = 0;
        bool sc_dst = false;
        bool fuse_next = false;
        bool fuse_feed_aff = false;
        bool fuse_keep_out1 = true;
        int Kpad = 0;
    };
  public:
    float* workspace() const { return partial_.as<float>(); }
    unsigned* error_record() const { return sk_rec_.p; }
  private:
    float* tensor_ptr(int t) const { return arena_.as<float>() + plan_.tensors[t].offset * (size_t)cap_; }
    Plan plan_;
    std::vector<DevOp> dev_;
    DevBuf params_, arena_, partial_, wino_v_, wino_m_, w36_bf_;
    bool bf16x2_ = false;
    size_t wino_maxc_ = 0;
    size_t wino_elems_ = 0;
    int cap_ = 0;
    struct SkRecord {
        unsigned* p = nullptr;
        int device = -1;
        SkRecord() = default;
        SkRecord(const SkRecord&) = delete;
        SkRecord& operator=(const SkRecord&) = delete;
        ~SkRecord();
    } sk_rec_;
    unsigned sk_gen_ = 0;
    bool stem_ok_ = false;
    bool front_ok_ = false;
};

int letterbox_plan(int rows, int cols, int in_w, int in_h, int* new_w, int* new_h, float* scale);

struct FrameIn {
    const uint8_t* bgr;
    int32_t rows, cols, step;
};
inline bool frame_empty(const FrameIn& f) { return !f.bgr || f.rows <= 0 || f.cols <= 0; }

class StagedTable {
  public:
    StagedTable() = default;
    StagedTable(const StagedTable&) = delete;
    StagedTable& operator=(const StagedTable&) = delete;
    ~StagedTable();
    void* stage(size_t bytes);
    void* send(size_t bytes, hipStream_t s);
    void* dev() const { return dev_.p; }

  private:
    static constexpr int kSlots = 4;
    struct Slot { void* p = nullptr; size_t bytes = 0; hipEvent_t ev = nullptr; bool pending = false; } slot_[kSlots];
    int next_ = 0, cur_ = 0;
    DevBuf dev_;
};

class FrameTable {
  public:
    const FrameDesc* upload(const FrameIn* frames, int n, int in_w, int in_h, hipStream_t s);
    const FrameDesc* table() const { return static_cast<const FrameDesc*>(st_.dev()); }
    const float* scales() const { return reinterpret_cast<const float*>(table() + n_); }
    int size() const { return n_; }

  private:
    int n_ = 0;
    StagedTable st_;
};

struct TilePlan {
    std::vector<FrameIn> view_frames;
    std::vector<ViewDesc> views;
    std::vector<FrameSeg> segs;
    size_t key_total = 0;
    int plan(const FrameIn* frames, int n, const Tiling& t, int in_w, int in_h, int cap, int max_views);
};
constexpr int kTileMaxViews = 256;

class TileTable {
  public:
    void upload(const TilePlan& p, hipStream_t s);
    const ViewDesc* views() const { return static_cast<const ViewDesc*>(st_.dev()); }
    const FrameSeg* segs() const { return reinterpret_cast<const FrameSeg*>(views() + V_); }

  private:
    int V_ = 0;
    StagedTable st_;
};

void postprocess_views(PostArgs a, int n_frames, const TileTable* tab, float nms_thr, int* sup, FaceRec* out, int max_out, int* counts,
                       hipStream_t s);

class Detector {
  public:
    explicit Detector(const std::string& onnx_path);
    void detect_dev(const uint8_t* frames, int n, int rows, int cols, int step, long stride, float score_thr, float nms_thr,
                    FaceRec* out, int max_out, int* counts, hipStream_t s);
    Net& net() { return net_; }
    int num_anchors() const { return anchors_; }
// ... 180 lines not shown
```

### facerecognizeonnx_amd/csrc/gemm_tile.h

```cpp
#pragma once
#include <hip/hip_runtime.h>

#include "kernels.h"

namespace fh {

typedef float v4f __attribute__((ext_vector_type(4)));
typedef float v16f __attribute__((ext_vector_type(16)));
typedef unsigned v4u __attribute__((ext_vector_type(4)));
typedef __bf16 bf16x8 __attribute__((ext_vector_type(8)));

__device__ __forceinline__ void lds_dma16(const float* src, void* dst) {
#if defined(__HIP_DEVICE_COMPILE__)
    __builtin_amdgcn_global_load_lds(src, (__attribute__((address_space(3))) void*)dst, 16, 0, 0);
#else
    (void)src; (void)dst;
#endif
}

template <typename I>
__device__ __forceinline__ int xcd_tile(const I block, const int nblocks) {
    const int q = nblocks >> 3, r8 = nblocks & 7, x = block & 7;
    return x * q + min(x, r8) + (int)(block >> 3);
}
// ... 31 lines not shown
}

template <int BN>
__device__ __forceinline__ void gemm_load_chunk(GemmSrc& s, const int buf, const bool a_live = true, const float* const a_dead = nullptr) {
    v4f* const dA = s.dA + buf * gemm_buf_slots<BN>();
    v4f* const dB = s.dB + buf * gemm_buf_slots<BN>();
#pragma unroll
    for (int i = 0; i < GEMM_BM / 32; ++i) lds_dma16(a_live ? s.a + i * s.a32 : a_dead, dA + i * 32 * 8);
#pragma unroll
    for (int i = 0; i < BN / 32; ++i) lds_dma16(s.b + i * s.b32, dB + i * 32 * 8);
    s.a += 32; s.b += 32;
}

template <int TN>
struct GemmFrag {
    v4f x, w[TN];
};
template <int TN>
__device__ __forceinline__ GemmFrag<TN> gemm_frag(const v4f* const tile, const GemmLane& l, const int s) {
    const v4f* const X = tile + l.wid * (32 * 8) + l.fr * 8;
    const v4f* const Wt = tile + GEMM_BM * 8 + l.fr * 8;
    const int col = (2 * s + l.fh2) ^ l.fsw;
    GemmFrag<TN> f;
    f.x = X[col];
#pragma unroll
    for (int j = 0; j < TN; ++j) f.w[j] = Wt[j * 32 * 8 + col];
    return f;
}

template <int BN, int ABL = 0>
__device__ __forceinline__ void gemm_chunk_f32(v16f (&acc)[BN / 32], GemmLds<BN>& lds, const int tile_buf, const bool more, GemmSrc& src,
                                               const GemmLane& l, const bool a_live = true, const float* const a_dead = nullptr,
                                               const GemmFrag<BN / 32>* const held = nullptr) {
    constexpr int TN = BN / 32;
    const int buf = (ABL & 1) ? 0 : tile_buf;
    if ((ABL & 1) == 0 && more) gemm_load_chunk<BN>(src, buf ^ 1, a_live, a_dead);
    const v4f* const tile = lds[buf];
#pragma unroll
    for (int s = 0; s < 4; ++s) {
        GemmFrag<TN> f;
        if constexpr ((ABL & 2) != 0) {
            f = *held;
#if defined(__HIP_DEVICE_COMPILE__)
            asm volatile("" : "+v"(f.x));
#endif
        } else {
            f = gemm_frag<TN>(tile, l, s);
        }
#pragma unroll
        for (int e = 0; e < 4; ++e)
#pragma unroll
            for (int j = 0; j < TN; ++j) acc[j] = __builtin_amdgcn_mfma_f32_32x32x2f32(f.w[j][e], f.x[e], acc[j], 0, 0, 0);
    }
    if constexpr ((ABL & 4) == 0) __syncthreads();
}

__device__ __forceinline__ void gemm_split_bf16(const v4u lo4, const v4u hi4, bf16x8& h, bf16x8& m) {
    const v4u hh = {__builtin_amdgcn_perm(lo4[1], lo4[0], 0x05040100u), __builtin_amdgcn_perm(lo4[3], lo4[2], 0x05040100u),
                    __builtin_amdgcn_perm(hi4[1], hi4[0], 0x05040100u), __builtin_amdgcn_perm(hi4[3], hi4[2], 0x05040100u)};
    const v4u mm = {__builtin_amdgcn_perm(lo4[1], lo4[0], 0x07060302u), __builtin_amdgcn_perm(lo4[3], lo4[2], 0x07060302u),
                    __builtin_amdgcn_perm(hi4[1], hi4[0], 0x07060302u), __builtin_amdgcn_perm(hi4[3], hi4[2], 0x07060302u)};
    h = __builtin_bit_cast(bf16x8, hh); m = __builtin_bit_cast(bf16x8, mm);
}
template <int TN>
__device__ __forceinline__ void gemm_mma_bf16x2(v16f (&acc)[TN], const v4f* const tile, const GemmLane& l) {
    const v4u* const X = reinterpret_cast<const v4u*>(tile) + l.wid * (32 * 8) + l.fr * 8;
    const v4u* const Wt = reinterpret_cast<const v4u*>(tile) + GEMM_BM * 8 + l.fr * 8;
#pragma unroll
    for (int ks = 0; ks < 2; ++ks) {
        const int c0 = (4 * ks + 2 * l.fh2) ^ l.fsw, c1 = (4 * ks + 2 * l.fh2 + 1) ^ l.fsw;
        bf16x8 xh, xm;
        gemm_split_bf16(X[c0], X[c1], xh, xm);
#pragma unroll
        for (int j = 0; j < TN; ++j) {
            bf16x8 wh, wm;
            gemm_split_bf16(Wt[j * 32 * 8 + c0], Wt[j * 32 * 8 + c1], wh, wm);
            acc[j] = __builtin_amdgcn_mfma_f32_32x32x16_bf16(wm, xh, acc[j], 0, 0, 0);
            acc[j] = __builtin_amdgcn_mfma_f32_32x32x16_bf16(wh, xm, acc[j], 0, 0, 0);
            acc[j] = __builtin_amdgcn_mfma_f32_32x32x16_bf16(wh, xh, acc[j], 0, 0, 0);
        }
    }
}

template <int TN, int JB>
struct GemmStore {
    static constexpr int W = JB * 32, PITCH = W + 4, RPI = 64 / (W / 4);
    static constexpr int NSTORE = (TN / JB) * (32 / RPI);
    static constexpr size_t BYTES = 4 * 32 * PITCH * sizeof(float);
    static_assert(TN % JB == 0, "store scratch");
};
template <int TN, int JB>
__device__ __forceinline__ void gemm_store_lines(const v16f (&acc)[TN], float* const scratch, float* __restrict__ M, const int N, const int m0,
                                                 const int n0, const int wid, const int lane) {
    using S = GemmStore<TN, JB>;
    const int fr = lane & 31, fh2 = lane >> 5;
    float* const blk = scratch + wid * 32 * S::PITCH;
    const int rr = lane / (S::W / 4), cq = lane % (S::W / 4);
#pragma unroll
    for (int h = 0; h < TN / JB; ++h) {
        wave_lds_order();
#pragma unroll
        for (int jj = 0; jj < JB; ++jj)
#pragma unroll
            for (int g = 0; g < 4; ++g) {
                const int j = h * JB + jj;
                *reinterpret_cast<v4f*>(blk + fr * S::PITCH + jj * 32 + 8 * g + 4 * fh2) = v4f{acc[j][4 * g], acc[j][4 * g + 1], acc[j][4 * g + 2], acc[j][4 * g + 3]};
            }
        wave_lds_order();
        float* const obase = M + (size_t)(m0 + wid * 32 + rr) * N + n0 + h * S::W + 4 * cq;
#pragma unroll
        for (int i = 0; i < 32 / S::RPI; ++i)
            *reinterpret_cast<v4f*>(obase + (size_t)i * S::RPI * N) = *reinterpret_cast<const v4f*>(blk + (rr + i * S::RPI) * S::PITCH + 4 * cq);
    }
}

}
```

### facerecognizeonnx_amd/csrc/kernels.h

```cpp
#pragma once
#include <hip/hip_runtime.h>

#include <cstdint>
#include <string>

#include <vector>

namespace fh {

void hip_check(hipError_t e, const char* what);
#define FH_HIP(x) ::fh::hip_check((x), #x)

#if defined(__HIPCC__)
__device__ __forceinline__ void wave_lds_order() {
#if defined(__HIP_DEVICE_COMPILE__)
    __builtin_amdgcn_fence(__ATOMIC_ACQ_REL, "wavefront");
    __builtin_amdgcn_wave_barrier();
#endif
}
#endif

struct KernelTimer {
    static constexpr int kTags = 13;
    bool enabled = false;
// ... 8 lines not shown
    std::vector<Rec> recs_;
    std::vector<hipEvent_t> pool_;
    hipEvent_t cur_ = nullptr;
    hipEvent_t take();
};


struct ConvArgs {
    const float* in;
    const float* wt;
    const float* bias;
    const float* slope;
    const float* res;
    float* out1;
    float* out2;
    const float* s2;
    const float* t2;
    float* slabs;
    const float* zeros;
    int B, H, W, Cin, Ho, Wo, Cout;
    int ks, stride, pad;
    int Kpad;
    int bias_cls;
    const float* sc_in;
    int sc_H, sc_W, sc_C, sc_stride;
    int act;
    int res_mode;
    const float* dw_w;
    const float* dw_b;
    int dw_act;
    int dw_stride;
    const uint8_t* u8_src;
    long u8_img_stride;
    int u8_step, u8_srcH, u8_srcW, u8_inH, u8_inW, u8_stride, stem_act;
    const float* stem_wf;
    const float* stem_bf;
    const unsigned* stem_wfrag;
    int no_prio;
    int no_pw;
    int n_outs;
    float* outs[3];
    int oc0[4];
    int oact[3];
    int sk_enable;
    int cus;
    int wt_group_rows;
    long wt_gs;
    double t_flops, t_bytes;
    int sk_full, sk_units, sk_q, sk_helpers, sk_rem, sk_owner_chunks, sk_maxp;
    unsigned* sk_err;
    int ep_direct;
    unsigned sk_timeout;
    int sk_test_drop;
    int tile0;
};

void launch_conv(const ConvArgs& a, int cfg, hipStream_t s);
int conv_pick_cfg(long M, int Cout);
void conv_workspace_init(float* ws);
void conv_workspace_reset_async(float* ws, hipStream_t s);
unsigned* conv_error_words();
unsigned* conv_error_record_new();
void conv_error_record_release(unsigned* r);
bool conv_take_error(std::string& msg, unsigned* rec);
bool conv_error_pending(const unsigned* rec);
unsigned conv_error_generation();
void conv_debug_streamk(int drop_publish, int timeout_ms);
unsigned conv_debug_generation();
size_t wino2_weight_floats(int Cin, int Cout);
void wino2_pack_weights(const float* w_ohwi, int Cout, int Cin, float* dst);
bool wino2_ok(const ConvArgs& a);
void launch_wino2(const ConvArgs& a, hipStream_t s);
long wino2_blocks(const ConvArgs& a);
double wino2_debug_clock_mhz();
const float* conv_zero_line();
int conv_num_cus();
bool conv_halo_ok(const ConvArgs& a);
size_t conv_halo_wfrag_floats(int Cin, int Cout);
void conv_halo_pack_weights(const float* w_ohwi, int Cout, int Cin, float* dst);
void launch_conv_halo(const ConvArgs& a, const float* wfrag, hipStream_t s);
bool front_fused_ok(int Cin, int Cout, int dw_stride);
void launch_dwpw(const ConvArgs& a, hipStream_t s);
void launch_conv_winograd(const ConvArgs& a, const float* wt36, float* V, float* M, int cfg, const float* in_scale, const float* in_shift,
                          hipStream_t s, bool bf16x2 = false);
struct WinoPlanes;
void launch_wino_input(const ConvArgs& a, float* V, const float* in_scale, const float* in_shift, bool pack, hipStream_t s);
void launch_wino_gemm(const ConvArgs& a, const float* wt36, const float* V, float* M, int cfg, bool bf16x2, hipStream_t s,
                      const WinoPlanes* mix = nullptr);
bool wino_gemm_ok_bf16x2(int Cin, int Cout);
void launch_wino_output(const ConvArgs& a, const float* M, hipStream_t s);
bool wino_can_fuse(int H, int W, int C, bool touches_memory);
void launch_wino_fused(const ConvArgs& a, const float* M, float* Vnext, int feed_aff, bool pack_next, hipStream_t s);
void launch_pack_bf16x2(const float* in, float* out, long n, hipStream_t s);
struct WinoPlanes {
    int e[4];
    int t[4];
    int nfc[4];
    int f2[4];
    int n[4];
    int rows[4];
    int base[4];
    int total_tiles;
    int planes;
};
bool wino_mix_layout(int B, int H, int W, int Cin, int Cout, WinoPlanes* out);
void launch_wino_mix(const ConvArgs& a, const WinoPlanes& pl, const float* M, float* Vnext, int feed_aff, const float* in_scale,
                     const float* in_shift, bool pack_next, hipStream_t s);
void wino_filter_transform(const double g[9], double u[36]);
void wino_debug_slots(int slots);
long wino_rows(long tiles);
int conv_wt_rows(int Cout);
size_t conv_slab_floats();
void conv_pack_weights(const float* w, int Cout, int Cin, int ks, float* dst);
inline int conv_kpad(int Ktot) { return (Ktot + 31) / 32 * 32; }

void launch_dwconv3x3(const float* in, const float* w9c, const float* bias, float* out, int B, int H, int W,
                      int C, int stride, int act, const float* slope, hipStream_t s);
void launch_dwglobal(const float* in, const float* w, const float* bias, float* out, int B, int taps, int C, int act, const float* slope,
                     hipStream_t s);
void launch_gconv3x3(const float* in, const float* w, const float* bias, float* out, int B, int H, int W, int C, int G, int stride, int act,
                     const float* slope, hipStream_t s);
void launch_affine(const float* in, const float* sc, const float* sh, float* out, long pixels, int C, hipStream_t s);
void launch_act(const float* in, const float* slope, float* out, long pixels, int C, int act, hipStream_t s);
void launch_add(const float* a, const float* b, float* out, long n, hipStream_t s);
void launch_upsample2x(const float* in, float* out, int B, int H, int W, int C, hipStream_t s);

struct FaceRec {
    int32_t x, y, w, h;
    float score;
    float lm[10];
};

void launch_det_preprocess(const uint8_t* frames, long img_stride, int rows, int cols, int step, int B,
                           int inH, int inW, int newH, int newW, float* out, hipStream_t s);
void launch_rec_preprocess(const uint8_t* crops, int n, int H, int W, float* out, hipStream_t s);

struct StemArgs {
    const uint8_t* src;
    long img_stride;
    int srcH, srcW, step, B;
    int inH, inW, stride, Cout;
    const float *w27, *bias;
    const float *wf, *biasf;
    const unsigned* wfrag;
    const float* slope;
    int act;
    float *out1, *out2;
    const float *s2, *t2;
    int cus;
};
void launch_stem(const StemArgs& a, hipStream_t s);
void stem_pack_wfrag(const float* wf, int Cout, unsigned* out);

struct ViewDesc {
    int32_t frame, local, x, y, w, h, edges;
    float scale;
};
static_assert(sizeof(ViewDesc) == 32, "ViewDesc is a 32-byte table row");
struct FrameSeg {
    int32_t first_view, views, key_off, seg_cap;
};
struct PostArgs {
    const float* score[3];
    const float* bbox[3];
    const float* kps[3];
    int inH, inW;
    const float* rows;
    int n_rows, feat;
    const ViewDesc* views;
    const FrameSeg* segs;
    const float* scales;
    float scale;
// ... 132 lines not shown
```

### facerecognizeonnx_amd/csrc/winograd.hip

```cpp
#include <hip/hip_runtime.h>

#include <algorithm>
#include <cstdlib>
#include <stdexcept>

#include "gemm_tile.h"
#include "kernels.h"
#include "plan.h"
#include "wino_xform.h"

namespace fh {

__global__ __launch_bounds__(256) void pack_bf16x2_kernel(const float* __restrict__ in, float* __restrict__ out, long n4) {
    for (long i = (long)blockIdx.x * blockDim.x + threadIdx.x; i < n4; i += (long)gridDim.x * blockDim.x)
        *reinterpret_cast<v4f*>(out + 4 * i) = wino_pack_bf16x2(*reinterpret_cast<const v4f*>(in + 4 * i));
}
void launch_pack_bf16x2(const float* in, float* out, long n, hipStream_t s) {
    const long n4 = n / 4;
    if (n4 > 0) hipLaunchKernelGGL(pack_bf16x2_kernel, dim3((unsigned)std::min<long>((n4 + 255) / 256, 256 * 64)), dim3(256), 0, s, in, out, n4);
}

__global__ __launch_bounds__(256, 2) void wino_input_kernel(const float* __restrict__ in, float* __restrict__ V, int B, int H, int W,
                                                            int C, int TY, int TX, long NTp, const float* __restrict__ aff_s,
                                                            const float* __restrict__ aff_t, const int pack) {
    const int C4 = C >> 2;
    const int NT = B * TY * TX;
    const int total = NT * C4;
    for (int idx = blockIdx.x * blockDim.x + threadIdx.x; idx < total; idx += gridDim.x * blockDim.x) {
        const int c4 = idx % C4;
        const int tile = idx / C4;
        const int tx = tile % TX, ty = (tile / TX) % TY, b = tile / (TX * TY);
        const int iy0 = 4 * ty - 1, ix0 = 4 * tx - 1;
        const float* img = in + (size_t)b * H * W * C + c4 * 4;
        v4f as4 = {1.f, 1.f, 1.f, 1.f}, at4 = {0.f, 0.f, 0.f, 0.f};
        if (aff_s) { as4 = *reinterpret_cast<const v4f*>(aff_s + c4 * 4); at4 = *reinterpret_cast<const v4f*>(aff_t + c4 * 4); }
        v4f t[6][6];
        v4f raw[6][6];
#pragma unroll
        for (int c = 0; c < 6; ++c) {
            const int ix = ix0 + c;
#pragma unroll
            for (int r = 0; r < 6; ++r) {
                const int iy = iy0 + r;
                raw[c][r] = *reinterpret_cast<const v4f*>(img + ((size_t)min(max(iy, 0), H - 1) * W + min(max(ix, 0), W - 1)) * C);
            }
        }
        __builtin_amdgcn_sched_barrier(0);
#pragma unroll
        for (int c = 0; c < 6; ++c) {
            const bool okx = (unsigned)(ix0 + c) < (unsigned)W;
            v4f d[6];
#pragma unroll
            for (int r = 0; r < 6; ++r) {
                const bool ok = okx && (unsigned)(iy0 + r) < (unsigned)H;
                v4f x;
#pragma unroll
                for (int e = 0; e < 4; ++e) x[e] = ok ? raw[c][r][e] : 0.f;
                d[r] = x * as4 + (ok ? at4 : v4f{0.f, 0.f, 0.f, 0.f});
            }
            v4f tc[6];
            wino_bt(d, tc);
#pragma unroll
            for (int i = 0; i < 6; ++i) t[i][c] = tc[i];
        }
        float* dst = V + (size_t)tile * C + c4 * 4;
        const size_t fs = (size_t)NTp * C;
        wino_input_rows<false>(t, false, pack, [&](int f, v4f o) { *reinterpret_cast<v4f*>(dst + (size_t)f * fs) = o; });
    }
}

__global__ __launch_bounds__(256, 2) void wino_output_kernel(const WinoOutArgs p) {
    const int C = p.C, C4 = C >> 2;
    const int NT = p.B * p.TY * p.TX;
    const int total = NT * C4;
    const size_t fs = (size_t)p.NTp * C;
    for (int idx = blockIdx.x * blockDim.x + threadIdx.x; idx < total; idx += gridDim.x * blockDim.x) {
        const int c4 = idx % C4;
        const int tile = idx / C4;
        const int tx = tile % p.TX, ty = (tile / p.TX) % p.TY, b = tile / (p.TX * p.TY);
        const float* src = p.M + (size_t)tile * C + c4 * 4;
        wino_output_phase<false, false, false>(
            p, b, ty, tx, c4, false, false, [&](int f) { return *reinterpret_cast<const v4f*>(src + (size_t)f * fs); }, [](int, int, v4f, v4f) {});
    }
}

struct WinoFuseArgs {
    WinoOutArgs o;
    float* V;
    int feed_aff;
    int csl4, pitch, img;
    int pack;
};

__global__ __launch_bounds__(256, 2) void wino_fused_kernel(const WinoFuseArgs a) {
    const WinoOutArgs& p = a.o;
    extern __shared__ v4f act[];
    const int C = p.C, TPI = p.TY * p.TX, IMG = a.img, HW = p.H * p.W, PITCH = a.pitch;
    const int tid = threadIdx.x, c4l = tid % a.csl4, slot = tid / a.csl4;
    const int cslices = C / (4 * a.csl4);
    const int cs = blockIdx.x % cslices, b0 = (blockIdx.x / cslices) * IMG;
    const int il = slot / TPI, tile = slot - il * TPI;
    const int ty = tile / p.TX, tx = tile - ty * p.TX;
// ... 44 lines not shown
    if (!live) return;
    const v4f* img = act + c4l;
    float* dst = a.V + tg * C + c4 * 4;
    wino_input_phase<false>(
        p.H, p.W, ty, tx, false, false, a.pack, [&](int iy, int ix) { return img[(iy * 32 + wino_slice_slot(ix & 31)) * 8]; },
        [&](int f, v4f o) { *reinterpret_cast<v4f*>(dst + (size_t)f * fs) = o; });
}

static int wino_slice_enabled() {
    static int v = -1;
    if (v < 0) { const char* e = getenv("FACEHIP_WINO_SLICE"); v = e ? atoi(e) : 1; }
    return v;
}
static bool wino_slice_shape(int H, int W, int C) {
    const int tpi = ((H + 3) / 4) * ((W + 3) / 4);
    return wino_slice_enabled() && C % 32 == 0 && tpi > 16 && tpi <= kSliceTiles && W <= 32 && (size_t)H * 32 * 8 * sizeof(v4f) <= 160 * 1024;
}


__device__ __forceinline__ int wino_plane_freq(const WinoPlanes& pl, const int tile_m) {
    const int c = tile_m >= pl.e[3] ? 3 : tile_m >= pl.e[2] ? 2 : tile_m >= pl.e[1] ? 1 : 0;
    const int pln = (tile_m - pl.e[c]) / pl.t[c];
    const int nfc = pl.nfc[c], f2 = pl.f2[c];
    int i = pln / nfc, j = pln - i * nfc;
    if ((f2 & 2) && i == 3) i = 5;
    if ((f2 & 1) && j == 3) j = 5;
    return 6 * i + j;
}

#ifdef FACEHIP_WINO_STAMP
__device__ unsigned long long g_wino_stamp[8 * 4096];
extern "C" __attribute__((visibility("default"))) int fh_debug_wino_stamps(unsigned long long* host, int n) {
    return hipMemcpyFromSymbol(host, HIP_SYMBOL(g_wino_stamp), sizeof(unsigned long long) * (size_t)(n < 8 * 4096 ? n : 8 * 4096)) == hipSuccess ? 0 : -1;
}
#define WINO_STAMP(i) if (threadIdx.x == 0 && blockIdx.x < 4096) g_wino_stamp[blockIdx.x * 8 + (i)] = __builtin_amdgcn_s_memrealtime()
#else
#define WINO_STAMP(i)
#endif
template <int BN, int OCC, int ABL = 0>
__global__ __launch_bounds__(256, OCC) void wino_gemm_kernel(const float* __restrict__ V, const float* __restrict__ U, float* __restrict__ M,
                                                            const int K, const int N, const WinoPlanes pl, const long wt_gs,
                                                            const int tiles_n, const int chunks) {
    constexpr int BM = GEMM_BM, TN = BN / 32, JB = TN >= 2 ? 2 : 1;
    __shared__ v4f lds[2][(BM + BN) * 8];
    WINO_STAMP(0);
    const GemmLane l = gemm_lane();
    const int tile = xcd_tile(blockIdx.x, gridDim.x);
    const int tile_n = tile % tiles_n, tile_m = tile / tiles_n;
    const int m0 = tile_m * BM, n0 = tile_n * BN;
    const float* Ug = U + (size_t)wino_plane_freq(pl, tile_m) * wt_gs;
    GemmSrc src = gemm_src<BN>(lds, V, m0, K, Ug, n0, K, l);
    v16f acc[TN];
#pragma unroll
    for (int j = 0; j < TN; ++j)
#pragma unroll
        for (int e = 0; e < 16; ++e) acc[j][e] = 0.f;
    gemm_load_chunk<BN>(src, 0);
    __syncthreads();
    WINO_STAMP(1);
    GemmFrag<TN> held{};
    if constexpr ((ABL & 2) != 0) held = gemm_frag<TN>(lds[0], l, 0);
    for (int kc = 0; kc < chunks; ++kc) gemm_chunk_f32<BN, ABL & 7>(acc, lds, kc & 1, kc + 1 < chunks, src, l, true, nullptr, &held);
    WINO_STAMP(2);
    if constexpr ((ABL & 8) != 0) { if (acc[0][0] != 123.456f) return; }
    if constexpr ((ABL & 16) == 0) {
        static_assert(GemmStore<TN, JB>::BYTES <= sizeof(lds), "store scratch");
        gemm_store_lines<TN, JB>(acc, reinterpret_cast<float*>(&lds[0][0]), M, N, m0, n0, l.wid, l.lane);
        WINO_STAMP(3);
#ifdef FACEHIP_WINO_STAMP
        asm volatile("s_waitcnt vmcnt(0)" ::: "memory");
        WINO_STAMP(4);
        if (l.tid == 0 && blockIdx.x < 4096) { g_wino_stamp[blockIdx.x * 8 + 5] = (unsigned long long)tile; g_wino_stamp[blockIdx.x * 8 + 6] = __builtin_amdgcn_s_getreg((3 << 11) | 20); }
#endif
    } else {
        float* orow = M + (size_t)(m0 + l.wid * 32 + l.fr) * N + n0 + 4 * l.fh2;
#pragma unroll
        for (int j = 0; j < TN; ++j)
#pragma unroll
            for (int g = 0; g < 4; ++g)
                *reinterpret_cast<v4f*>(orow + j * 32 + 8 * g) = v4f{acc[j][4 * g], acc[j][4 * g + 1], acc[j][4 * g + 2], acc[j][4 * g + 3]};
    }
}

template <int BN, int OCC>
__global__ __launch_bounds__(256, OCC) void wino_gemm_pers_kernel(const float* __restrict__ V, const float* __restrict__ U, float* __restrict__ M,
                                                                 const int K, const int N, const WinoPlanes pl, const long wt_gs,
                                                                 const int tiles_n, const int chunks, const int ntiles) {
    constexpr int BM = GEMM_BM, TN = BN / 32;
    constexpr int BUF = gemm_buf_slots<BN>();
    __shared__ v4f lds[2][BUF];
    const GemmLane l = gemm_lane();
    auto tile_of = [&](int vb) { return xcd_tile(vb, ntiles); };
    GemmSrc src;
    auto point_at = [&](int tile) {
        const int tile_n = tile % tiles_n, tile_m = tile / tiles_n;
        const float* Ug = U + (size_t)wino_plane_freq(pl, tile_m) * wt_gs;
        src = gemm_src<BN>(lds, V, tile_m * BM, K, Ug, tile_n * BN, K, l);
    };
    using Store = GemmStore<TN, 1>;
    static_assert(Store::BYTES <= BUF * sizeof(v4f), "store scratch must fit ONE tile buffer");
    int base = 0;
    int vb = blockIdx.x;
    point_at(tile_of(vb));
    gemm_load_chunk<BN>(src, 0);
    __syncthreads();
    for (;;) {
        const int tile = tile_of(vb);
        const int m0 = (tile / tiles_n) * BM, n0 = (tile % tiles_n) * BN;
        v16f acc[TN];
#pragma unroll
        for (int j = 0; j < TN; ++j)
#pragma unroll
            for (int e = 0; e < 16; ++e) acc[j][e] = 0.f;
        for (int kc = 0; kc < chunks; ++kc) gemm_chunk_f32<BN>(acc, lds, (base + kc) & 1, kc + 1 < chunks, src, l);
        const int last = (base + chunks - 1) & 1;
        const int nvb = vb + gridDim.x;
        const bool more = nvb < ntiles;
        if (more) {
            point_at(tile_of(nvb));
            gemm_load_chunk<BN>(src, last ^ 1);
#if defined(__HIP_DEVICE_COMPILE__)
            __builtin_amdgcn_sched_barrier(0);
#endif
        }
        gemm_store_lines<TN, 1>(acc, reinterpret_cast<float*>(&lds[last][0]), M, N, m0, n0, l.wid, l.lane);
        if (!more) break;
        vb = nvb; base = last ^ 1;
#if defined(__HIP_DEVICE_COMPILE__)
        asm volatile("s_waitcnt vmcnt(%0) lgkmcnt(0)" ::"n"(Store::NSTORE) : "memory");
        __builtin_amdgcn_s_barrier();
        __builtin_amdgcn_sched_barrier(0);
#endif
    }
}

template <int BN, int OCC>
__global__ __launch_bounds__(256, OCC) void wino_gemm_bf16x2_kernel(const float* __restrict__ V, const float* __restrict__ U, float* __restrict__ M,
                                                                   const int K, const int N, const WinoPlanes pl, const long wt_gs,
                                                                   const int tiles_n, const int chunks) {
    constexpr int BM = GEMM_BM, TN = BN / 32, JB = TN >= 2 ? 2 : 1;
    __shared__ v4f lds[2][(BM + BN) * 8];
    const GemmLane l = gemm_lane();
    const int tile = xcd_tile(blockIdx.x, gridDim.x);
    const int tile_n = tile % tiles_n, tile_m = tile / tiles_n;
    const int m0 = tile_m * BM, n0 = tile_n * BN;
    const float* Ug = U + (size_t)wino_plane_freq(pl, tile_m) * wt_gs;
    GemmSrc src = gemm_src<BN>(lds, V, m0, K, Ug, n0, K, l);
    v16f acc[TN];
#pragma unroll
    for (int j = 0; j < TN; ++j)
#pragma unroll
        for (int e = 0; e < 16; ++e) acc[j][e] = 0.f;
    gemm_load_chunk<BN>(src, 0);
    __syncthreads();
    for (int kc = 0; kc < chunks; ++kc) {
        const int buf = kc & 1;
        if (kc + 1 < chunks) gemm_load_chunk<BN>(src, buf ^ 1);
        gemm_mma_bf16x2<TN>(acc, lds[buf], l);
        __syncthreads();
    }
    static_assert(GemmStore<TN, JB>::BYTES <= sizeof(lds), "store scratch");
    gemm_store_lines<TN, JB>(acc, reinterpret_cast<float*>(&lds[0][0]), M, N, m0, n0, l.wid, l.lane);
}

long wino_rows(long tiles) { return (tiles + 255) / 256 * 256; }

static inline int wino_grid(long n) {
    const long b = (n + 255) / 256;
    return (int)(b < 1 ? 1 : b > 256 * 16 ? 256 * 16 : b);
}

void wino_filter_transform(const double g[9], double u[36]) {
    static const double G[6][3] = {{1.0 / 4, 0, 0},          {-1.0 / 6, -1.0 / 6, -1.0 / 6}, {-1.0 / 6, 1.0 / 6, -1.0 / 6},
                                   {1.0 / 24, 1.0 / 12, 1.0 / 6}, {1.0 / 24, -1.0 / 12, 1.0 / 6},  {0, 0, 1}};
    double t[6][3];
    for (int i = 0; i < 6; ++i)
        for (int kx = 0; kx < 3; ++kx) t[i][kx] = G[i][0] * g[0 * 3 + kx] + G[i][1] * g[1 * 3 + kx] + G[i][2] * g[2 * 3 + kx];
    for (int i = 0; i < 6; ++i)
        for (int j = 0; j < 6; ++j) u[i * 6 + j] = t[i][0] * G[j][0] + t[i][1] * G[j][1] + t[i][2] * G[j][2];
}

static void wino_check(long NT, int cmax) {
    if (NT * (cmax / 4) >= (1L << 31) || 36 * (NT + 256) >= (1L << 31))
        throw std::runtime_error("winograd: batch too large for the 32-bit tile index (split the batch)");
}

bool wino_gemm_ok_bf16x2(int Cin, int Cout) { return Cout % 64 == 0 && Cin % 32 == 0; }

static int g_wino_slots_override = 0;
void wino_debug_slots(int slots) { g_wino_slots_override = slots > 0 ? (slots + 7) / 8 * 8 : 0; }
static long wino_slots(int occ, int cus) {
    if (g_wino_slots_override) return g_wino_slots_override;
    const long s = (long)occ * (cus > 0 ? cus : 256) / 8 * 8;
    return s < 8 ? 8 : s;
}

static int wino_pers_enabled() {
    static int v = -1;
    if (v < 0) { const char* e = getenv("FACEHIP_WINO_PERS"); v = e ? atoi(e) : 0; }
    return v || g_wino_slots_override;
}

static int wino_mix_enabled() {
    static int v = -1;
    if (v < 0) { const char* e = getenv("FACEHIP_WINO_MIX"); v = e ? atoi(e) : 1; }
    return v;
}

static bool wino_bn128(bool mixed) {
    static int v = -1;
    if (v < 0) { const char* e = getenv("FACEHIP_WINO_BN128"); v = e ? atoi(e) : 1; }
    return v == 2 || (v == 1 && mixed);
}

static bool wino_pick_bn128(long row_tiles, int Cout, bool mixed, int cus) {
    static const int force = [] { const char* e = getenv("FACEHIP_WINO_BN128"); return e ? atoi(e) : -1; }();
    if (force >= 0) return wino_bn128(mixed);
    const long sw = wino_slots(2, cus), sn = wino_slots(3, cus);
    const long wide = (row_tiles * (Cout / 128) + sw - 1) / sw * 4, narrow = (row_tiles * (Cout / 64) + sn - 1) / sn * 3;
    if (wide != narrow) return wide < narrow;
    return wino_bn128(mixed);
}

bool wino_mix_layout(int B, int H, int W, int Cin, int Cout, WinoPlanes* out) {
    const int TY = (H + 3) / 4, TX = (W + 3) / 4;
    const int my = (H & 3) == 1 || (H & 3) == 2, mx = (W & 3) == 1 || (W & 3) == 2;
    if (!wino_mix_enabled() || !(my || mx) || TY * TX != 16 || Cin % 64 || Cout % 64 || B < 64) return false;
    if ((size_t)H * W * 16 * sizeof(v4f) > 64 * 1024) return false;
    WinoPlanes pl{};
    const int n[4] = {(TY - my) * (TX - mx), (TY - my) * mx, my * (TX - mx), my * mx};
    int tile = 0, row = 0, planes = 0;
    for (int c = 0; c < 4; ++c) {
        const int nfr = (c & 2) ? 4 : 6, nfc = (c & 1) ? 4 : 6;
        pl.n[c] = n[c]; pl.nfc[c] = nfc; pl.f2[c] = c;
        pl.rows[c] = (B * n[c] + 127) / 128 * 128;
        pl.t[c] = pl.rows[c] / 128;
        pl.e[c] = tile; pl.base[c] = row;
        tile += nfr * nfc * pl.t[c]; row += nfr * nfc * pl.rows[c];
        if (n[c]) planes += nfr * nfc;
    }
    if ((long)row * std::max(Cin, Cout) * 4 >= (1L << 31)) return false;
    pl.total_tiles = tile; pl.planes = planes;
    if (out) *out = pl;
    return true;
}

void launch_wino_gemm(const ConvArgs& a, const float* wt36, const float* V, float* M, int cfg, bool bf16x2, hipStream_t s, const WinoPlanes* mix) {
    const int TY = (a.H + 3) / 4, TX = (a.W + 3) / 4;
    const long NT = (long)a.B * TY * TX;
    if (NT <= 0) return;
    const long NTp = wino_rows(NT);
    KernelTimer& timer = KernelTimer::get();
    ConvArgs g{};
    g.in = V; g.wt = wt36; g.out1 = M; g.slabs = a.slabs; g.sk_err = a.sk_err; g.sk_enable = a.sk_enable; g.cus = a.cus;
    g.B = (int)(36 * NTp); g.H = g.W = g.Ho = g.Wo = 1; g.Cin = a.Cin; g.Cout = a.Cout; g.ks = 1; g.stride = 1; g.pad = 0; g.Kpad = a.Cin;
    g.act = (int)Act::NONE; g.res_mode = (int)ResMode::NONE;
    g.wt_group_rows = (int)NTp; g.wt_gs = (long)conv_wt_rows(a.Cout) * a.Cin;
    g.t_flops = 2.0 * 36.0 * (double)NT * a.Cin * a.Cout; g.t_bytes = a.t_flops;
    WinoPlanes pl{};
    if (mix) {
        if (!(a.Cout % 32 == 0 && cfg == 2)) throw std::runtime_error("winograd: the mixed tiling runs on the lean GEMM kernel only");
        pl = *mix;
        double real_rows = 0;
        for (int c = 0; c < 4; ++c) real_rows += (double)((c & 2) ? 4 : 6) * pl.nfc[c] * a.B * pl.n[c];
        g.t_flops = 2.0 * real_rows * a.Cin * a.Cout;
    } else {
        pl.e[0] = 0; pl.e[1] = pl.e[2] = pl.e[3] = (int)(36 * NTp / 128); pl.t[0] = (int)(NTp / 128); pl.nfc[0] = 6;
        pl.total_tiles = pl.e[1];
    }
    if (a.Cout % 32 == 0 && cfg == 2) {
        const long row_tiles = pl.total_tiles;
        const int chunks = a.Cin / 32;
        const bool wide = a.Cout % 64 == 0;
        using TileKernel = void (*)(const float*, const float*, float*, int, int, WinoPlanes, long, int, int);
        auto launch = [&](TileKernel kernel, int BN) {
            hipLaunchKernelGGL(kernel, dim3((unsigned)(row_tiles * (a.Cout / BN))), dim3(256), 0, s, V, wt36, M, a.Cin, a.Cout, pl, g.wt_gs, a.Cout / BN, chunks);
        };
        auto launch_pers = [&](auto kernel, int BN, int OCC) {
            const long nt = row_tiles * (a.Cout / BN), slots = wino_slots(OCC, a.cus);
            if (!wino_pers_enabled() || nt <= slots) return false;
            hipLaunchKernelGGL(kernel, dim3((unsigned)slots), dim3(256), 0, s, V, wt36, M, a.Cin, a.Cout, pl, g.wt_gs, a.Cout / BN, chunks, (int)nt);
            return true;
        };
        timer.begin(s);
        if (bf16x2) {
            if (!wino_gemm_ok_bf16x2(a.Cin, a.Cout)) throw std::runtime_error("winograd: this layer has no split-bf16 GEMM");
            launch(wino_gemm_bf16x2_kernel<64, 3>, 64);
        } else if (wide && a.Cout % 128 == 0 && wino_pick_bn128(row_tiles, a.Cout, mix != nullptr, a.cus)) {
            if (!launch_pers(wino_gemm_pers_kernel<128, 2>, 128, 2)) launch(wino_gemm_kernel<128, 2>, 128);
        } else if (wide) {
            if (!launch_pers(wino_gemm_pers_kernel<64, 3>, 64, 3)) {
#ifdef FACEHIP_WINO_ABL
                static const int abl = [] { const char* e = getenv("FACEHIP_WINO_ABL"); return e ? atoi(e) : 0; }();
#define WABL(X) case X: launch(wino_gemm_kernel<64, 3, X>, 64); break;
                switch (abl) { WABL(1) WABL(2) WABL(3) WABL(4) WABL(5) WABL(6) WABL(7) WABL(8) WABL(15) WABL(16) WABL(17) WABL(24)
                    default: launch(wino_gemm_kernel<64, 3>, 64); }
#undef WABL
#else
                launch(wino_gemm_kernel<64, 3>, 64);
#endif
            }
        } else
            launch(wino_gemm_kernel<32, 4>, 32);
        timer.end(s, 7, g.t_flops, g.t_bytes);
    } else {
        if (bf16x2) throw std::runtime_error("winograd: this layer has no split-bf16 GEMM");
        launch_conv(g, cfg, s);
    }
}

static WinoOutArgs wino_out_args(const ConvArgs& a, const float* M) {
    const int TY = (a.H + 3) / 4, TX = (a.W + 3) / 4;
    WinoOutArgs o{};
    o.M = M; o.bias = a.bias; o.slope = a.slope; o.res = a.res; o.out1 = a.out1; o.out2 = a.out2; o.s2 = a.s2; o.t2 = a.t2;
    o.B = a.B; o.H = a.H; o.W = a.W; o.C = a.Cout; o.TY = TY; o.TX = TX; o.act = a.act; o.NTp = wino_rows((long)a.B * TY * TX);
    return o;
}

template <class Kernel, class... Args>
static void launch_wino_xform(Kernel kernel, dim3 grid, dim3 block, size_t lds, hipStream_t s, const Args&... args) {
    KernelTimer& timer = KernelTimer::get();
    timer.begin(s);
    hipLaunchKernelGGL(kernel, grid, block, lds, s, args...);
    timer.end(s, 8, 0.0, 0.0);
}

void launch_wino_input(const ConvArgs& a, float* V, const float* in_scale, const float* in_shift, bool pack, hipStream_t s) {
    const int TY = (a.H + 3) / 4, TX = (a.W + 3) / 4;
    const long NT = (long)a.B * TY * TX;
    if (NT <= 0) return;
    wino_check(NT, std::max(a.Cin, a.Cout));
    launch_wino_xform(wino_input_kernel, dim3(wino_grid(NT * (a.Cin >> 2))), dim3(256), 0, s, a.in, V, a.B, a.H, a.W, a.Cin, TY, TX, wino_rows(NT),
                      in_scale, in_shift, pack ? 1 : 0);
}

void launch_wino_output(const ConvArgs& a, const float* M, hipStream_t s) {
    const WinoOutArgs o = wino_out_args(a, M);
    const long NT = (long)a.B * o.TY * o.TX;
    if (NT <= 0) return;
    launch_wino_xform(wino_output_kernel, dim3(wino_grid(NT * (a.Cout >> 2))), dim3(256), 0, s, o);
}

static bool wino_fuse_shape(int H, int W, int C, int* csl4, int* pitch, int* img) {
    const int tpi = ((H + 3) / 4) * ((W + 3) / 4);
    int c = 0, pt = 0, im = 0;
    if (C % 64 == 0 && tpi <= 16 && (tpi & (tpi - 1)) == 0) { c = 16; pt = 16; im = 16 / tpi; }
    else if (C % 16 == 0 && tpi <= 64) { c = 4; pt = 5; im = 64 / tpi; }
    else return false;
    if ((size_t)im * H * W * pt * sizeof(v4f) > 64 * 1024) return false;
    if (csl4) { *csl4 = c; *pitch = pt; *img = im; }
    return true;
}
bool wino_can_fuse(int H, int W, int C, bool touches_memory) {
    if (wino_slice_shape(H, W, C)) return true;
    int csl4 = 0, pitch = 0, img = 0;
    if (!wino_fuse_shape(H, W, C, &csl4, &pitch, &img)) return false;
    return csl4 == 16 || !touches_memory;
}

void launch_wino_fused(const ConvArgs& a, const float* M, float* Vnext, int feed_aff, bool pack_next, hipStream_t s) {
    const bool slice = wino_slice_shape(a.H, a.W, a.Cout);
    WinoFuseArgs f{};
    f.csl4 = 8; f.pitch = 8; f.img = 1;
    if (!slice && !wino_fuse_shape(a.H, a.W, a.Cout, &f.csl4, &f.pitch, &f.img)) throw std::runtime_error("winograd: this map cannot take the fused transform");
    f.o = wino_out_args(a, M);
    f.V = Vnext; f.feed_aff = feed_aff; f.pack = pack_next ? 1 : 0;
    const long NT = (long)a.B * f.o.TY * f.o.TX;
    if (NT <= 0) return;
    wino_check(NT, a.Cout);
    if (slice) {
        static const bool attr = [] {
            FH_HIP(hipFuncSetAttribute(reinterpret_cast<const void*>(&wino_slice_kernel), hipFuncAttributeMaxDynamicSharedMemorySize, 160 * 1024));
            return true;
        }();
        (void)attr;
        launch_wino_xform(wino_slice_kernel, dim3((unsigned)(a.B * (a.Cout / 32))), dim3(kSliceThreads), (size_t)a.H * 32 * 8 * sizeof(v4f), s, f);
    } else {
        launch_wino_xform(wino_fused_kernel, dim3((unsigned)(((a.B + f.img - 1) / f.img) * (a.Cout / (4 * f.csl4)))), dim3(256),
                          (size_t)f.img * a.H * a.W * f.pitch * sizeof(v4f), s, f);
    }
}

struct WinoMixArgs {
    WinoOutArgs o;
    WinoPlanes pl;
    const float* in; const float* in_s; const float* in_t;
    float* V;
    unsigned plane_bytes;
    int feed_aff, pack;
};

__global__ __launch_bounds__(256, 2) void wino_mix_kernel(const WinoMixArgs a) {
    const WinoOutArgs& p = a.o;
    extern __shared__ v4f act[];
    const int C = p.C, HW = p.H * p.W;
    const int tid = threadIdx.x, c4l = tid & 15, tile = tid >> 4;
    const int cslices = C >> 6;
    const int cs = blockIdx.x % cslices, b = blockIdx.x / cslices;
    const int ty = tile / p.TX, tx = tile - ty * p.TX;
    const int my = a.pl.n[2] + a.pl.n[3] > 0, mx = a.pl.n[1] + a.pl.n[3] > 0;
    const bool rF2 = my && ty == p.TY - 1, cF2 = mx && tx == p.TX - 1;
    const int nfr = rF2 ? 4 : 6, nfc = cF2 ? 4 : 6;
    const int n_c = rF2 ? (cF2 ? a.pl.n[3] : a.pl.n[2]) : (cF2 ? a.pl.n[1] : a.pl.n[0]);
    const int rows_c = rF2 ? (cF2 ? a.pl.rows[3] : a.pl.rows[2]) : (cF2 ? a.pl.rows[1] : a.pl.rows[0]);
    const int base_c = rF2 ? (cF2 ? a.pl.base[3] : a.pl.base[2]) : (cF2 ? a.pl.base[1] : a.pl.base[0]);
    const int lidx = rF2 ? (cF2 ? 0 : tx) : (cF2 ? ty : ty * (p.TX - mx) + tx);
    const int c4 = cs * 16 + c4l;
    const unsigned off0 = (unsigned)(((base_c + b * n_c + lidx) * C + c4 * 4) * 4);
    const unsigned pstride = (unsigned)rows_c * (unsigned)C * 4u;
    auto plane_off = [&](int f) {
        const int i = f / 6, j = f % 6;
        return i < nfr && j < nfc ? off0 + (unsigned)(i * nfc + j) * pstride : 0x80000000u;
    };
    if (p.M) {
        const __amdgpu_buffer_rsrc_t rm = __builtin_amdgcn_make_buffer_rsrc(const_cast<float*>(p.M), 0, a.plane_bytes, 0x00020000);
        wino_output_phase<true, true, true>(
            p, b, ty, tx, c4, rF2, cF2, [&](int f) { return __builtin_bit_cast(v4f, __builtin_amdgcn_raw_buffer_load_b128(rm, plane_off(f), 0, 0)); },
            [&](int oy, int ox, v4f v, v4f vb) { act[(oy * p.W + ox) * 16 + c4l] = a.feed_aff ? vb : v; });
    } else {
        v4f as4 = {1.f, 1.f, 1.f, 1.f}, at4 = {0.f, 0.f, 0.f, 0.f};
        if (a.in_s) { as4 = *reinterpret_cast<const v4f*>(a.in_s + c4 * 4); at4 = *reinterpret_cast<const v4f*>(a.in_t + c4 * 4); }
        const float* src = a.in + (size_t)b * HW * C + c4 * 4;
        for (int px = tile; px < HW; px += 16) act[px * 16 + c4l] = *reinterpret_cast<const v4f*>(src + (size_t)px * C) * as4 + at4;
    }
    if (!a.V) return;
    __syncthreads();
    const __amdgpu_buffer_rsrc_t rv = __builtin_amdgcn_make_buffer_rsrc(a.V, 0, a.plane_bytes, 0x00020000);
    const v4f* img = act + c4l;
    wino_input_phase<true>(
        p.H, p.W, ty, tx, rF2, cF2, a.pack, [&](int iy, int ix) { return img[(iy * p.W + ix) * 16]; },
        [&](int f, v4f o) { __builtin_amdgcn_raw_buffer_store_b128(__builtin_bit_cast(v4u, o), rv, plane_off(f), 0, 0); });
}

void launch_wino_mix(const ConvArgs& a, const WinoPlanes& pl, const float* M, float* Vnext, int feed_aff, const float* in_scale,
                     const float* in_shift, bool pack_next, hipStream_t s) {
    if (a.B <= 0) return;
    WinoMixArgs f{};
    f.o = wino_out_args(a, M);
    if (!M) { f.o.C = a.Cin; f.o.res = nullptr; f.o.out1 = f.o.out2 = nullptr; }
    f.pl = pl;
    f.in = a.in; f.in_s = in_scale; f.in_t = in_shift;
    f.V = Vnext; f.feed_aff = feed_aff; f.pack = pack_next ? 1 : 0;
    long rows = 0;
    for (int c = 0; c < 4; ++c) rows += (long)((c & 2) ? 4 : 6) * pl.nfc[c] * pl.rows[c];
    f.plane_bytes = (unsigned)(rows * f.o.C * 4);
    if (f.o.C % 64 || f.o.TY * f.o.TX != 16 || rows * f.o.C * 4 >= (1L << 31)) throw std::runtime_error("winograd: this map cannot take the mixed tiling");
    launch_wino_xform(wino_mix_kernel, dim3((unsigned)(a.B * (f.o.C / 64))), dim3(256), (size_t)a.H * a.W * 16 * sizeof(v4f), s, f);
}

void launch_conv_winograd(const ConvArgs& a, const float* wt36, float* V, float* M, int cfg, const float* in_scale, const float* in_shift,
                          hipStream_t s, bool bf16x2) {
    WinoPlanes pl;
    if (cfg == 2 && wino_mix_layout(a.B, a.H, a.W, a.Cin, a.Cout, &pl)) {
        launch_wino_mix(a, pl, nullptr, V, 0, in_scale, in_shift, bf16x2, s);
        launch_wino_gemm(a, wt36, V, M, cfg, bf16x2, s, &pl);
        launch_wino_mix(a, pl, M, nullptr, 0, nullptr, nullptr, false, s);
        return;
    }
    launch_wino_input(a, V, in_scale, in_shift, bf16x2, s);
    launch_wino_gemm(a, wt36, V, M, cfg, bf16x2, s);
    launch_wino_output(a, M, s);
}

}
```

### include/facehip.h

```cpp
#ifndef FACEHIP_H_
#define FACEHIP_H_

#include <stddef.h>
#include <stdint.h>

#ifdef __cplusplus
extern "C" {
#endif

#define FH_API __attribute__((visibility("default")))

enum fh_status { FH_OK = 0, FH_ERR_ARG = -1, FH_ERR_MODEL = -2, FH_ERR_DEVICE = -3, FH_ERR_STATE = -4 };

typedef struct fh_face {
    int32_t x, y, w, h;
    float score;
    float lm[10];
} fh_face;

typedef struct fh_det fh_det;
typedef struct fh_rec fh_rec;
typedef struct fh_gallery fh_gallery;

FH_API const char* fh_version(void);
// ... 162 lines not shown
FH_API int fh_gallery_get_scan(const fh_gallery* g);
FH_API int fh_gallery_scan_stats(fh_gallery* g, long long* certified, long long* fallback);
FH_API int fh_topk_merge_dev(const float* d_part_scores, const int* d_part_idx, int nparts, int nq, int k, float* d_scores,
                             int* d_indices, void* stream);
#define FH_COMM_ID_BYTES 128
typedef struct fh_comm fh_comm;
FH_API int fh_comm_unique_id(unsigned char id[FH_COMM_ID_BYTES]);
FH_API fh_comm* fh_comm_create(int rank, int world, const unsigned char id[FH_COMM_ID_BYTES], int device);
FH_API void fh_comm_destroy(fh_comm* c);
FH_API int fh_comm_rank(const fh_comm* c);
FH_API int fh_comm_world(const fh_comm* c);
FH_API int fh_comm_allgather_f32_dev(fh_comm* c, const float* d_send, float* d_recv, long long count, void* stream);
FH_API int fh_gallery_topk_sharded_dev(fh_gallery* g, fh_comm* c, const float* d_queries_local, int nq_local, int k,
                                       float* d_scores, int* d_indices, void* stream);
FH_API long long fh_gallery_enroll(fh_gallery* g, const float* rows, long long n, int rows_on_device);
FH_API long long fh_gallery_size(fh_gallery* g);
FH_API int fh_gallery_label_dev(fh_gallery* g, const float* d_queries, int nq, float threshold, int* d_labels,
                                float* d_scores, void* stream);

FH_API long long fh_gallery_enroll_ids(fh_gallery* g, const float* rows, const int* ids, long long n, int on_device);
FH_API int fh_gallery_upload_ids(fh_gallery* g, const float* rows, const int* ids, long long n, int on_device, long long index_base);
FH_API int fh_gallery_topk_ids_dev(fh_gallery* g, const float* d_queries, int nq, int k, float* d_scores, int* d_ids, int* d_rows,
                                   void* stream);
FH_API int fh_gallery_label_ids_dev(fh_gallery* g, const float* d_queries, int nq, float threshold, int* d_ids_out, float* d_scores,
                                    void* stream);
FH_API long long fh_gallery_remove_ids(fh_gallery* g, const int* ids_host, long long n_ids);
FH_API long long fh_gallery_get_ids(fh_gallery* g, long long first, long long n, int* ids_host_out);
FH_API int fh_topk_merge_ids_dev(const float* d_part_scores, const int* d_part_ids, const int* d_part_rows, int nparts, int nq, int k,
                                 float* d_scores, int* d_ids, int* d_rows, void* stream);

#define FH_FUSE_CHUNK 512
enum fh_gallery_fuse { FH_FUSE_UNIT = 0, FH_FUSE_SUM = 1 };
FH_API long long fh_gallery_group_ids(const int* ids, long long n, int* order, long long* starts, int* uniq);
FH_API long long fh_gallery_fuse_ids(fh_gallery* src, fh_gallery* dst, int mode);
FH_API long long fh_gallery_get_rows(fh_gallery* g, long long first, long long n, float* rows_host_out);
FH_API int fh_gallery_self_scores_dev(fh_gallery* src, fh_gallery* tmpl, float* d_scores, void* stream);

enum fh_cluster_noise { FH_CLUSTER_NOISE_NONE = 0, FH_CLUSTER_NOISE_SELF = 1 };
FH_API int fh_cluster_scores(const float* scores, int n, float threshold, int min_pts, int noise, int* labels, int* info);
FH_API int fh_gallery_cluster_dev(fh_gallery* g, float threshold, int min_pts, int noise, int* d_labels, int* d_info, void* stream);
FH_API long long fh_gallery_set_ids(fh_gallery* g, const int* ids, int on_device);

#define FH_HIST_BINS 2048
typedef struct fh_roc_point {
    float threshold;
    int32_t bin;
    unsigned long long true_accepts, false_accepts, genuine, impostor;
} fh_roc_point;
FH_API int fh_hist_bin(float score);
FH_API int fh_roc_from_hist(const unsigned long long* hist, double max_far, fh_roc_point out[2]);
FH_API int fh_gallery_pair_hist_dev(fh_gallery* g, unsigned long long* d_hist, unsigned long long* d_nan, void* stream);

#define FH_TAG_ALL 0xFFFFFFFFu
FH_API long long fh_gallery_set_tags(fh_gallery* g, long long first, long long n, const uint32_t* tags, int on_device);
FH_API long long fh_gallery_get_tags(fh_gallery* g, long long first, long long n, uint32_t* tags_host_out);
FH_API int fh_gallery_topk_tagged_dev(fh_gallery* g, const float* d_queries, const uint32_t* d_masks, int nq, int k, float* d_scores,
                                      int* d_indices, void* stream);
FH_API int fh_gallery_topk_ids_tagged_dev(fh_gallery* g, const float* d_queries, const uint32_t* d_masks, int nq, int k, float* d_scores,
                                          int* d_ids, int* d_rows, void* stream);
FH_API int fh_gallery_label_tagged_dev(fh_gallery* g, const float* d_queries, const uint32_t* d_masks, int nq, float threshold,
                                       int* d_labels, float* d_scores, void* stream);
FH_API int fh_gallery_label_ids_tagged_dev(fh_gallery* g, const float* d_queries, const uint32_t* d_masks, int nq, float threshold,
                                           int* d_ids_out, float* d_scores, void* stream);
FH_API int fh_gallery_tag_stats(fh_gallery* g, long long* tiles_scanned, long long* tiles_skipped);
FH_API int fh_tracker_set_stream_masks(fh_tracker* t, const uint32_t* masks_host );

#define FH_RANGE_MAX_CAP 1024
FH_API int fh_gallery_range_dev(fh_gallery* g, const float* d_queries, const uint32_t* d_masks , int nq, float threshold,
                                int cap, long long* d_counts , float* d_scores ,
                                int* d_indices , int* d_ids , void* stream);
FH_API int fh_range_from_scores(const float* scores, long long n, long long index_base, const uint32_t* tags , uint32_t mask,
                                float threshold, int cap, long long* count, float* out_scores, int* out_indices);

FH_API int fh_timing_enable(int on);
FH_API int fh_timing_num_tags(void);
FH_API int fh_timing_collect(double* ms, double* flops, double* bytes, long long* launches, int n);
FH_API int fh_timing_collect_ops(double* ms, double* flops, int* tag, int cap);
FH_API int fh_det_set_conv_cfg(fh_det* d, int cfg, int stream_k);
FH_API int fh_rec_set_conv_cfg(fh_rec* r, int cfg, int stream_k);
FH_API int fh_det_set_winograd(fh_det* d, int on);
FH_API int fh_rec_set_winograd(fh_rec* r, int on);
FH_API int fh_rec_set_wino_fusion(fh_rec* r, int on);
FH_API int fh_rec_set_shortcut_fold(fh_rec* r, int on);
enum fh_precision { FH_PREC_FP32 = 0, FH_PREC_BF16X2 = 1 };
FH_API int fh_rec_set_precision(fh_rec* r, int mode, float* worst);
FH_API int fh_rec_get_precision(fh_rec* r);
FH_API int fh_det_set_cus(fh_det* d, int cus);
FH_API int fh_rec_set_cus(fh_rec* r, int cus);
FH_API int fh_det_set_fused_stem(fh_det* d, int on);
FH_API int fh_rec_set_fused_stem(fh_rec* r, int on);
FH_API int fh_det_set_fused_front(fh_det* d, int on);
FH_API int fh_det_set_halo_conv(fh_det* d, int on);

FH_API int fh_imread(const char* path, unsigned char** bgr, int* rows, int* cols);
FH_API int fh_image_decode(const unsigned char* bytes, size_t n, unsigned char** bgr, int* rows, int* cols);
FH_API void fh_image_free(unsigned char* bgr);

FH_API int fh_memcpy_d2h(void* host_dst, const void* dev_src, size_t bytes);
FH_API int fh_resize_u8c3_dev(const uint8_t* d_src, int sh, int sw, int sstep, uint8_t* d_dst, int dh, int dw, int dstep,
                              void* stream);
FH_API int fh_conv_forward_dev(const float* d_in, const float* d_wt_packed, const float* d_bias, float* d_out, int batch,
                               int h, int w, int cin, int cout, int ksize, int stride, int kpad, int cfg, void* stream);
FH_API int fh_conv_winograd_dev(const float* d_in, const float* w_ohwi_host, const float* d_bias, float* d_out, int batch, int h, int w,
                                int cin, int cout, void* stream);
FH_API int fh_conv_winograd_ex_dev(const float* d_in, const float* w_ohwi_host, const float* d_bias, float* d_out, int batch, int h, int w,
                                   int cin, int cout, int precision, void* stream);
FH_API int fh_conv_wino2_dev(const float* d_in, const float* w_ohwi_host, const float* d_bias, const float* d_slope, const float* d_res,
                             float* d_out, int batch, int h, int w, int cin, int cout, int act, int bias_cls, void* stream);
FH_API int fh_conv_wino2_ex_dev(const float* d_in, const float* w_ohwi_host, const float* d_bias, const float* d_slope, const float* d_res,
                                float* d_out, float* d_out2, const float* d_s2, const float* d_t2, int n_outs, float* const* d_outs,
                                const int* oc0, const int* oact, int batch, int h, int w, int cin, int cout, int act, int bias_cls,
                                void* stream);
FH_API double fh_debug_wino2_clock_mhz(void);
FH_API int fh_set_graph_replay(int on);
FH_API const float* fh_det_workspace_dev(fh_det* d);
FH_API int fh_det_graph_stats(fh_det* d, long long* replays);
FH_API int fh_rec_graph_stats(fh_rec* r, long long* replays);
FH_API int fh_debug_streamk(int drop_publish, int timeout_ms);
FH_API int fh_debug_wino_slots(int slots);
FH_API int fh_debug_cluster_tiles(int tiles_per_wg);
FH_API int fh_debug_hist_copies(int copies);
FH_API int fh_debug_tag_skip(int on);
FH_API int fh_debug_pack_bf16x2_dev(const float* d_in, float* d_out, long long n);
FH_API long long fh_debug_wino_gemm_rows(int batch, int h, int w, int k, int n, int mixed);
FH_API int fh_debug_wino_gemm_dev(const float* d_V, const float* d_U, float* d_M, int batch, int h, int w, int k, int n, int precision,
                                  int mixed, void* stream);
FH_API int fh_debug_topk_merge_strided_dev(const float* d_ps, const int* d_pi, int nparts, int nq, int k, long long part_stride,
                                           float* d_scores, int* d_indices, void* stream);
FH_API int fh_conv_wt_rows(int cout);
FH_API int fh_conv_pack_weights(const float* w_ohwi, int cout, int cin, int ksize, float* dst_packed);
FH_API int fh_conv_kpad(int ktot);

#ifdef __cplusplus
}
#endif
#endif
```

Baseline: 12510 faces/s.

## Add three-piece bf16 split Winograd GEMM for fp32-accurate recognizer convs

Adds an x3 precision mode for the recognizer's Winograd GEMM. Activations are split on the fly into three bf16 pieces, weights are pre-packed into three bf16 planes, and six bf16 MFMA products are accumulated to emulate fp32 accuracy. It is enabled by default through an environment switch and applies to every eligible layer, replacing the fp32 GEMM path. The aim is to move fp32 Winograd GEMM work onto bf16 matrix cores. The cost is six MFMAs per step, extra LDS traffic for the three weight planes, and extra weight memory.

```diff
diff --git a/facerecognizeonnx_amd/_lib.py b/facerecognizeonnx_amd/_lib.py
--- a/facerecognizeonnx_amd/_lib.py
+++ b/facerecognizeonnx_amd/_lib.py
@@ -217,6 +217,8 @@
     "fh_det_set_winograd": (_i, [_vp, _i]),
     "fh_rec_set_winograd": (_i, [_vp, _i]),
     "fh_rec_set_wino_fusion": (_i, [_vp, _i]),
+    "fh_rec_set_wino_x3": (_i, [_vp, _i]),
+    "fh_rec_get_wino_x3": (_i, [_vp]),
     "fh_rec_set_shortcut_fold": (_i, [_vp, _i]),
     "fh_rec_set_precision": (_i, [_vp, _i, C.POINTER(C.c_float)]),
     "fh_rec_get_precision": (_i, [_vp]),
diff --git a/facerecognizeonnx_amd/api.py b/facerecognizeonnx_amd/api.py
--- a/facerecognizeonnx_amd/api.py
+++ b/facerecognizeonnx_amd/api.py
@@ -246,6 +246,9 @@
         worst = C.c_float(0.0)
         check(_lib.lib().fh_rec_set_precision(self._h, modes[mode], C.byref(worst)), "fh_rec_set_precision")
         return float(worst.value)
+
+    def set_wino_x3(self, on: bool = True) -> int:
+        return check(_lib.lib().fh_rec_set_wino_x3(self._h, 1 if on else 0), "fh_rec_set_wino_x3")
 
     def precision(self) -> str:
         return "bf16x2" if _lib.lib().fh_rec_get_precision(self._h) == 1 else "fp32"
diff --git a/facerecognizeonnx_amd/csrc/api.cpp b/facerecognizeonnx_amd/csrc/api.cpp
--- a/facerecognizeonnx_amd/csrc/api.cpp
+++ b/facerecognizeonnx_amd/csrc/api.cpp
@@ -1467,6 +1467,12 @@
 }
 int fh_det_set_winograd(fh_det* d, int on) { if (!d) return arg_error("null handle"); d->det.net().winograd = on != 0; return FH_OK; }
 int fh_rec_set_winograd(fh_rec* r, int on) { if (!r) return arg_error("null handle"); r->rec.net().winograd = on != 0; return FH_OK; }
+int fh_rec_set_wino_x3(fh_rec* r, int on) {
+    if (!r) return arg_error("null handle");
+    Owns owns(&r->rec.net());
+    return guarded([&] { return r->rec.net().set_wino_x3(on != 0, nullptr); });
+}
+int fh_rec_get_wino_x3(fh_rec* r) { return r && r->rec.net().wino_x3() ? 1 : 0; }
 int fh_rec_set_wino_fusion(fh_rec* r, int on) { if (!r) return arg_error("null handle"); r->rec.net().fuse_wino = on != 0; return FH_OK; }
 int fh_rec_set_precision(fh_rec* r, int mode, float* worst_out) {
     if (!r || (mode != FH_PREC_FP32 && mode != FH_PREC_BF16X2)) return arg_error("fh_rec_set_precision: bad argument");
@@ -1549,12 +1555,12 @@
 }
 int fh_conv_winograd_ex_dev(const float* d_in, const float* w_ohwi, const float* d_bias, float* d_out, int batch, int h, int w, int cin,
                             int cout, int precision, void* stream) {
-    if (!d_in || !w_ohwi || !d_out || cin % 32 || cout % 4 || (precision != FH_PREC_FP32 && precision != FH_PREC_BF16X2))
+    if (!d_in || !w_ohwi || !d_out || cin % 32 || cout % 4 || (precision != FH_PREC_FP32 && precision != FH_PREC_BF16X2 && precision != FH_PREC_F32X3))
         return arg_error("fh_conv_winograd_dev: bad argument");
-    const bool bf2 = precision == FH_PREC_BF16X2;
+    const bool bf2 = precision == FH_PREC_BF16X2, x3 = precision == FH_PREC_F32X3;
     Owns owns(nullptr);
     return guarded([&] {
-        if (bf2 && !fh::wino_gemm_ok_bf16x2(cin, cout)) throw std::runtime_error("winograd: this layer has no split-bf16 GEMM");
+        if ((bf2 || x3) && !fh::wino_gemm_ok_bf16x2(cin, cout)) throw std::runtime_error("winograd: this layer has no split-bf16 GEMM");
         const int rows = fh::conv_wt_rows(cout);
         std::vector<float> u36((size_t)36 * rows * cin, 0.f), uf((size_t)cout * cin);
         std::vector<double> uall((size_t)cout * cin * 36);
@@ -1578,6 +1584,9 @@
         if (bf2) {
             dUp.ensure(u36.size() * sizeof(float));
             fh::launch_pack_bf16x2(dU.as<float>(), dUp.as<float>(), (long)u36.size(), S(stream));
+        } else if (x3) {
+            dUp.ensure(36 * fh::wino_x3_floats(rows, cin) * sizeof(float));
+            fh::launch_pack_x3(dU.as<float>(), dUp.as<float>(), rows, cin, S(stream));
         }
         static fh::DevBuf slabs;
         static unsigned slabs_gen = 0;
@@ -1587,7 +1596,7 @@
         a.in = d_in; a.bias = d_bias; a.out1 = d_out; a.slabs = slabs.as<float>(); a.sk_enable = 1;
         a.B = batch; a.H = h; a.W = w; a.Ho = h; a.Wo = w; a.Cin = cin; a.Cout = cout; a.ks = 3; a.stride = 1; a.pad = 1;
         a.act = (int)fh::Act::NONE; a.res_mode = (int)fh::ResMode::NONE;
-        fh::launch_conv_winograd(a, (bf2 ? dUp : dU).as<float>(), dV.as<float>(), dM.as<float>(), 2, nullptr, nullptr, S(stream), bf2);
+        fh::launch_conv_winograd(a, (bf2 || x3 ? dUp : dU).as<float>(), dV.as<float>(), dM.as<float>(), 2, nullptr, nullptr, S(stream), precision);
         FH_HIP(hipStreamSynchronize(S(stream)));
         return 0;
     });
@@ -1621,27 +1630,30 @@
 }
 int fh_debug_wino_gemm_dev(const float* d_V, const float* d_U, float* d_M, int batch, int h, int w, int k, int n, int precision, int mixed,
                            void* stream) {
-    if (!d_V || !d_U || !d_M || (precision != FH_PREC_FP32 && precision != FH_PREC_BF16X2))
+    if (!d_V || !d_U || !d_M || (precision != FH_PREC_FP32 && precision != FH_PREC_BF16X2 && precision != FH_PREC_F32X3))
         return arg_error("fh_debug_wino_gemm_dev: bad argument");
     fh::WinoPlanes pl{};
     const long long rows = wino_gemm_rows(batch, h, w, k, n, mixed, &pl);
     if (rows == -2) return arg_error("fh_debug_wino_gemm_dev: the mixed tiling does not apply to this layer");
     if (rows < 0) return arg_error("fh_debug_wino_gemm_dev: bad argument (k % 32 == 0, n % 32 == 0)");
-    const bool bf2 = precision == FH_PREC_BF16X2;
+    const bool bf2 = precision == FH_PREC_BF16X2, x3 = precision == FH_PREC_F32X3;
     Owns owns(nullptr);
     return guarded([&] {
-        if (bf2 && !fh::wino_gemm_ok_bf16x2(k, n)) throw std::runtime_error("winograd: this layer has no split-bf16 GEMM");
+        if ((bf2 || x3) && !fh::wino_gemm_ok_bf16x2(k, n)) throw std::runtime_error("winograd: this layer has no split-bf16 GEMM");
         const size_t nv = (size_t)rows * k, nu = (size_t)36 * fh::conv_wt_rows(n) * k;
         fh::DevBuf dVp, dUp;
         if (bf2) {
             dVp.ensure(nv * sizeof(float)); dUp.ensure(nu * sizeof(float));
             fh::launch_pack_bf16x2(d_V, dVp.as<float>(), (long)nv, S(stream));
             fh::launch_pack_bf16x2(d_U, dUp.as<float>(), (long)nu, S(stream));
+        } else if (x3) {
+            dUp.ensure(36 * fh::wino_x3_floats(fh::conv_wt_rows(n), k) * sizeof(float));
+            fh::launch_pack_x3(d_U, dUp.as<float>(), fh::conv_wt_rows(n), k, S(stream));
         }
         fh::ConvArgs a{};
         a.B = batch; a.H = h; a.W = w; a.Ho = h; a.Wo = w; a.Cin = k; a.Cout = n; a.ks = 3; a.stride = 1; a.pad = 1;
         a.act = (int)fh::Act::NONE; a.res_mode = (int)fh::ResMode::NONE;
-        fh::launch_wino_gemm(a, bf2 ? dUp.as<float>() : d_U, bf2 ? dVp.as<float>() : d_V, d_M, 2, bf2, S(stream), mixed ? &pl : nullptr);
+        fh::launch_wino_gemm(a, bf2 || x3 ? dUp.as<float>() : d_U, bf2 ? dVp.as<float>() : d_V, d_M, 2, precision, S(stream), mixed ? &pl : nullptr);
         FH_HIP(hipGetLastError());
         FH_HIP(hipStreamSynchronize(S(stream)));
         return 0;
diff --git a/facerecognizeonnx_amd/csrc/engine.cpp b/facerecognizeonnx_amd/csrc/engine.cpp
--- a/facerecognizeonnx_amd/csrc/engine.cpp
+++ b/facerecognizeonnx_amd/csrc/engine.cpp
@@ -201,6 +201,7 @@
                 }
                 d.w36 = push(u36.data(), u36.size());
                 d.w36n = u36.size();
+                d.w36k = op.Cin;
                 d.wino = true;
                 d.bf2 = wino_gemm_ok_bf16x2(op.Cin, op.Cout);
                 const size_t tiles = (size_t)((op.H + 3) / 4) * ((op.W + 3) / 4);
@@ -391,6 +392,21 @@
         FH_HIP(hipStreamSynchronize(s));
     }
     bf16x2_ = on && layers > 0;
+    return on ? layers : 0;
+}
+
+int Net::set_wino_x3(bool on, hipStream_t s) {
+    int layers = 0;
+    size_t total = 0;
+    for (auto& d : dev_)
+        if (d.wino && d.bf2) { d.w36x = total; total += 36 * wino_x3_floats((int)(d.w36n / 36 / d.w36k), d.w36k); ++layers; }
+    if (on && layers > 0 && w36_x3_.bytes < total * sizeof(float)) {
+        w36_x3_.ensure(total * sizeof(float));
+        for (const auto& d : dev_)
+            if (d.wino && d.bf2) launch_pack_x3(params_.as<float>() + d.w36, w36_x3_.as<float>() + d.w36x, (int)(d.w36n / 36 / d.w36k), d.w36k, s);
+        FH_HIP(hipStreamSynchronize(s));
+    }
+    wino_x3_ = on && layers > 0;
     return on ? layers : 0;
 }
 
@@ -468,6 +484,9 @@
                     const bool bf2 = bf16x2_ && d.bf2 && force_cfg < 0;
                     WinoPlanes pl;
                     const bool mix = wcfg == 2 && wino_mix_layout(batch, op.H, op.W, op.Cin, op.Cout, &pl);
+                    const long row_tiles = mix ? pl.total_tiles : 36 * wino_rows((long)batch * ((op.H + 3) / 4) * ((op.W + 3) / 4)) / 128;
+                    const bool x3 = !bf2 && wino_x3_ && d.bf2 && force_cfg < 0 && wcfg == 2 && wino_x3_pays(row_tiles, op.Cin, op.Cout);
+                    const float* const u36 = bf2 ? w36_bf_.as<float>() + d.w36p : x3 ? w36_x3_.as<float>() + d.w36x : P + d.w36;
                     if (!v_ready) {
                         const float* in_s = nullptr; const float* in_t = nullptr;
                         if (d.aff_src >= 0) {
@@ -477,8 +496,7 @@
                         if (mix) launch_wino_mix(a, pl, nullptr, wino_v_.as<float>(), 0, in_s, in_t, bf2, s);
                         else launch_wino_input(a, wino_v_.as<float>(), in_s, in_t, bf2, s);
                     }
-                    launch_wino_gemm(a, bf2 ? w36_bf_.as<float>() + d.w36p : P + d.w36, wino_v_.as<float>(), wino_m_.as<float>(), wcfg, bf2, s,
-                                     mix ? &pl : nullptr);
+                    launch_wino_gemm(a, u36, wino_v_.as<float>(), wino_m_.as<float>(), wcfg, bf2 ? 1 : x3 ? 2 : 0, s, mix ? &pl : nullptr);
                     v_ready = false;
                     if (d.fuse_next && fuse_wino && i + 1 < plan_.ops.size()) {
                         const POp& nx = plan_.ops[i + 1];
@@ -818,6 +836,7 @@
 Recognizer::Recognizer(const std::string& onnx_path) : net_(onnx_path, 112, 112) {
     const auto& o = net_.plan().outputs.at(0);
     dim_ = o.rows * o.cols;
+    if (wino_x3_default()) net_.set_wino_x3(true, nullptr);
 }
 
 void Recognizer::embed_aligned_dev(const uint8_t* crops, int n, float* out, hipStream_t s, float* raw_out) {
diff --git a/facerecognizeonnx_amd/csrc/engine.h b/facerecognizeonnx_amd/csrc/engine.h
--- a/facerecognizeonnx_amd/csrc/engine.h
+++ b/facerecognizeonnx_amd/csrc/engine.h
@@ -56,13 +56,15 @@
     bool fuse_wino = true;
     int set_bf16x2(bool on, hipStream_t s);
     bool bf16x2() const { return bf16x2_; }
+    int set_wino_x3(bool on, hipStream_t s);
+    bool wino_x3() const { return wino_x3_; }
     int cus = 0;
     int force_cfg = -1;
     bool sk_enable = true;
     long long config_word() const {
         return (long long)fuse_stem | (long long)fuse_front << 1 | (long long)winograd << 2 | (long long)halo_conv << 3 |
                (long long)fold_shortcut << 4 | (long long)fuse_wino << 5 | (long long)bf16x2_ << 6 | (long long)sk_enable << 7 |
-               (long long)(cus & 0xffff) << 8 | (long long)((force_cfg + 1) & 0xff) << 24;
+               (long long)(cus & 0xffff) << 8 | (long long)((force_cfg + 1) & 0xff) << 24 | (long long)wino_x3_ << 32;
     }
 
   private:
@@ -75,6 +77,8 @@
         size_t dww = 0, dwb = 0;
         size_t w36 = 0;
         size_t w36n = 0, w36p = 0;
+        size_t w36x = 0;
+        int w36k = 0;
         bool bf2 = false;
         size_t wfrag = 0;
         bool halo = false;
@@ -101,8 +105,8 @@
     float* tensor_ptr(int t) const { return arena_.as<float>() + plan_.tensors[t].offset * (size_t)cap_; }
     Plan plan_;
     std::vector<DevOp> dev_;
-    DevBuf params_, arena_, partial_, wino_v_, wino_m_, w36_bf_;
-    bool bf16x2_ = false;
+    DevBuf params_, arena_, partial_, wino_v_, wino_m_, w36_bf_, w36_x3_;
+    bool bf16x2_ = false, wino_x3_ = false;
     size_t wino_maxc_ = 0;
     size_t wino_elems_ = 0;
     int cap_ = 0;
diff --git a/facerecognizeonnx_amd/csrc/gemm_tile.h b/facerecognizeonnx_amd/csrc/gemm_tile.h
--- a/facerecognizeonnx_amd/csrc/gemm_tile.h
+++ b/facerecognizeonnx_amd/csrc/gemm_tile.h
@@ -137,6 +137,89 @@
     }
 }
 
+typedef float v2f_ __attribute__((ext_vector_type(2)));
+typedef __bf16 bf16x2_ __attribute__((ext_vector_type(2)));
+__device__ __forceinline__ void gemm_split3(const v4f lo4, const v4f hi4, bf16x8& h, bf16x8& m, bf16x8& l) {
+    v4u hw, mw, lw;
+#pragma unroll
+    for (int p = 0; p < 4; ++p) {
+        const float a = p < 2 ? lo4[2 * p] : hi4[2 * p - 4], b = p < 2 ? lo4[2 * p + 1] : hi4[2 * p - 3];
+        const unsigned ab = __builtin_bit_cast(unsigned, a), bb = __builtin_bit_cast(unsigned, b);
+        hw[p] = __builtin_amdgcn_perm(bb, ab, 0x07060302u);
+        const v2f_ r = {a - __builtin_bit_cast(float, ab & 0xffff0000u), b - __builtin_bit_cast(float, bb & 0xffff0000u)};
+        mw[p] = __builtin_bit_cast(unsigned, __builtin_convertvector(r, bf16x2_));
+        const v2f_ q = {r[0] - __builtin_bit_cast(float, mw[p] << 16), r[1] - __builtin_bit_cast(float, mw[p] & 0xffff0000u)};
+        lw[p] = __builtin_bit_cast(unsigned, __builtin_convertvector(q, bf16x2_));
+    }
+    h = __builtin_bit_cast(bf16x8, hw); m = __builtin_bit_cast(bf16x8, mw); l = __builtin_bit_cast(bf16x8, lw);
+}
+
+template <int BN> constexpr int gemm_buf_slots_x3() { return GEMM_BM * 8 + 3 * BN * 4; }
+template <int BN> using GemmLdsX3 = v4f[2][gemm_buf_slots_x3<BN>()];
+struct GemmSrcX3 {
+    const float* a;
+    const v4f* b;
+    size_t a32, bplane, bchunk;
+    v4f* dA;
+    v4f* dB;
+};
+template <int BN>
+__device__ __forceinline__ GemmSrcX3 gemm_src_x3(GemmLdsX3<BN>& lds, const float* A, const int m0, const int lda, const float* B3, const int n0,
+                                                 const int brows, const int chunks, const GemmLane& l) {
+    return GemmSrcX3{A + (size_t)(m0 + l.lrow()) * lda + l.lqs() * 4, reinterpret_cast<const v4f*>(B3) + (size_t)n0 * 4 + l.tid, (size_t)32 * lda,
+                     (size_t)chunks * brows * 4, (size_t)brows * 4, &lds[0][l.wid * 64], &lds[0][GEMM_BM * 8 + l.wid * 64]};
+}
+template <int BN>
+__device__ __forceinline__ void gemm_load_chunk_x3(GemmSrcX3& s, const int buf) {
+    v4f* const dA = s.dA + buf * gemm_buf_slots_x3<BN>();
+    v4f* const dB = s.dB + buf * gemm_buf_slots_x3<BN>();
+#pragma unroll
+    for (int i = 0; i < GEMM_BM / 32; ++i) lds_dma16(s.a + i * s.a32, dA + i * 32 * 8);
+#pragma unroll
+    for (int p = 0; p < 3; ++p)
+#pragma unroll
+        for (int i = 0; i < BN / 64; ++i) lds_dma16(reinterpret_cast<const float*>(s.b + p * s.bplane + i * 256), dB + p * BN * 4 + i * 256);
+    s.a += 32; s.b += s.bchunk;
+}
+template <int TN>
+__device__ __forceinline__ void gemm_mma_x3(v16f (&acc)[TN], const v4f* const tile, const GemmLane& l) {
+    constexpr int PL = TN * 32 * 4;
+    const v4f* const X = tile + l.wid * (32 * 8) + l.fr * 8;
+    const v4f* const Wt = tile + GEMM_BM * 8 + l.fr * 4;
+    const int wsw = (l.fr >> 2) & 3;
+#pragma unroll
+    for (int ks = 0; ks < 2; ++ks) {
+        const int c0 = (4 * ks + 2 * l.fh2) ^ l.fsw, c1 = (4 * ks + 2 * l.fh2 + 1) ^ l.fsw;
+        const int wc = (2 * ks + l.fh2) ^ wsw;
+        bf16x8 xh, xm, xl, wh[TN], wm[TN], wl[TN];
+#pragma unroll
+        for (int j = 0; j < TN; ++j) {
+            wh[j] = __builtin_bit_cast(bf16x8, Wt[j * 32 * 4 + wc]);
+            wm[j] = __builtin_bit_cast(bf16x8, Wt[PL + j * 32 * 4 + wc]);
+            wl[j] = __builtin_bit_cast(bf16x8, Wt[2 * PL + j * 32 * 4 + wc]);
+        }
+        gemm_split3(X[c0], X[c1], xh, xm, xl);
+#pragma unroll
+        for (int j = 0; j < TN; ++j) acc[j] = __builtin_amdgcn_mfma_f32_32x32x16_bf16(wl[j], xh, acc[j], 0, 0, 0);
+#pragma unroll
+        for (int j = 0; j < TN; ++j) acc[j] = __builtin_amdgcn_mfma_f32_32x32x16_bf16(wh[j], xl, acc[j], 0, 0, 0);
+#pragma unroll
+        for (int j = 0; j < TN; ++j) acc[j] = __builtin_amdgcn_mfma_f32_32x32x16_bf16(wm[j], xm, acc[j], 0, 0, 0);
+#pragma unroll
+        for (int j = 0; j < TN; ++j) acc[j] = __builtin_amdgcn_mfma_f32_32x32x16_bf16(wm[j], xh, acc[j], 0, 0, 0);
+#pragma unroll
+        for (int j = 0; j < TN; ++j) acc[j] = __builtin_amdgcn_mfma_f32_32x32x16_bf16(wh[j], xm, acc[j], 0, 0, 0);
+#pragma unroll
+        for (int j = 0; j < TN; ++j) acc[j] = __builtin_amdgcn_mfma_f32_32x32x16_bf16(wh[j], xh, acc[j], 0, 0, 0);
+    }
+}
+template <int BN>
+__device__ __forceinline__ void gemm_chunk_x3(v16f (&acc)[BN / 32], GemmLdsX3<BN>& lds, const int buf, const bool more, GemmSrcX3& src, const GemmLane& l) {
+    if (more) gemm_load_chunk_x3<BN>(src, buf ^ 1);
+    gemm_mma_x3<BN / 32>(acc, lds[buf], l);
+    __syncthreads();
+}
+
 template <int TN, int JB>
 struct GemmStore {
     static constexpr int W = JB * 32, PITCH = W + 4, RPI = 64 / (W / 4);
diff --git a/facerecognizeonnx_amd/csrc/kernels.h b/facerecognizeonnx_amd/csrc/kernels.h
--- a/facerecognizeonnx_amd/csrc/kernels.h
+++ b/facerecognizeonnx_amd/csrc/kernels.h
@@ -114,12 +114,16 @@
 bool front_fused_ok(int Cin, int Cout, int dw_stride);
 void launch_dwpw(const ConvArgs& a, hipStream_t s);
 void launch_conv_winograd(const ConvArgs& a, const float* wt36, float* V, float* M, int cfg, const float* in_scale, const float* in_shift,
-                          hipStream_t s, bool bf16x2 = false);
+                          hipStream_t s, int prec = 0);
 struct WinoPlanes;
 void launch_wino_input(const ConvArgs& a, float* V, const float* in_scale, const float* in_shift, bool pack, hipStream_t s);
-void launch_wino_gemm(const ConvArgs& a, const float* wt36, const float* V, float* M, int cfg, bool bf16x2, hipStream_t s,
+void launch_wino_gemm(const ConvArgs& a, const float* wt36, const float* V, float* M, int cfg, int prec, hipStream_t s,
                       const WinoPlanes* mix = nullptr);
 bool wino_gemm_ok_bf16x2(int Cin, int Cout);
+void launch_pack_x3(const float* in, float* out, int rows, int K, hipStream_t s);
+inline size_t wino_x3_floats(int rows, int K) { return (size_t)rows * K * 3 / 2; }
+bool wino_x3_default();
+bool wino_x3_pays(long row_tiles, int Cin, int Cout);
 void launch_wino_output(const ConvArgs& a, const float* M, hipStream_t s);
 bool wino_can_fuse(int H, int W, int C, bool touches_memory);
 void launch_wino_fused(const ConvArgs& a, const float* M, float* Vnext, int feed_aff, bool pack_next, hipStream_t s);
diff --git a/facerecognizeonnx_amd/csrc/winograd.hip b/facerecognizeonnx_amd/csrc/winograd.hip
--- a/facerecognizeonnx_amd/csrc/winograd.hip
+++ b/facerecognizeonnx_amd/csrc/winograd.hip
@@ -3,6 +3,7 @@
 #include <algorithm>
 #include <cstdlib>
 #include <stdexcept>
+#include <type_traits>
 
 #include "gemm_tile.h"
 #include "kernels.h"
@@ -18,6 +19,23 @@
 void launch_pack_bf16x2(const float* in, float* out, long n, hipStream_t s) {
     const long n4 = n / 4;
     if (n4 > 0) hipLaunchKernelGGL(pack_bf16x2_kernel, dim3((unsigned)std::min<long>((n4 + 255) / 256, 256 * 64)), dim3(256), 0, s, in, out, n4);
+}
+
+__global__ __launch_bounds__(256) void wino_pack_x3_kernel(const float* __restrict__ in, v4u* __restrict__ out, int rows, int K, long n8) {
+    const int k8n = K >> 3, chunks = K >> 5;
+    for (long i = (long)blockIdx.x * 256 + threadIdx.x; i < n8; i += (long)gridDim.x * 256) {
+        const int k8 = (int)(i % k8n), n = (int)(i / k8n % rows), f = (int)(i / k8n / rows);
+        const float* src = in + ((size_t)f * rows + n) * K + 8 * k8;
+        bf16x8 h, m, l;
+        gemm_split3(*reinterpret_cast<const v4f*>(src), *reinterpret_cast<const v4f*>(src + 4), h, m, l);
+        const size_t plane = (size_t)chunks * rows * 4;
+        v4u* o = out + (size_t)f * 3 * plane + ((size_t)(k8 >> 2) * rows + n) * 4 + ((k8 & 3) ^ ((n >> 2) & 3));
+        o[0] = __builtin_bit_cast(v4u, h); o[plane] = __builtin_bit_cast(v4u, m); o[2 * plane] = __builtin_bit_cast(v4u, l);
+    }
+}
+void launch_pack_x3(const float* in, float* out, int rows, int K, hipStream_t s) {
+    const long n8 = 36L * rows * (K / 8);
+    if (n8 > 0) hipLaunchKernelGGL(wino_pack_x3_kernel, dim3((unsigned)std::min<long>((n8 + 255) / 256, 256 * 64)), dim3(256), 0, s, in, reinterpret_cast<v4u*>(out), rows, K, n8);
 }
 
 __global__ __launch_bounds__(256, 2) void wino_input_kernel(const float* __restrict__ in, float* __restrict__ V, int B, int H, int W,
@@ -228,27 +246,29 @@
     }
 }
 
-template <int BN, int OCC>
+template <int BN, int OCC, bool X3 = false>
 __global__ __launch_bounds__(256, OCC) void wino_gemm_pers_kernel(const float* __restrict__ V, const float* __restrict__ U, float* __restrict__ M,
                                                                  const int K, const int N, const WinoPlanes pl, const long wt_gs,
                                                                  const int tiles_n, const int chunks, const int ntiles) {
     constexpr int BM = GEMM_BM, TN = BN / 32;
-    constexpr int BUF = gemm_buf_slots<BN>();
+    constexpr int BUF = X3 ? gemm_buf_slots_x3<BN>() : gemm_buf_slots<BN>();
     __shared__ v4f lds[2][BUF];
     const GemmLane l = gemm_lane();
     auto tile_of = [&](int vb) { return xcd_tile(vb, ntiles); };
-    GemmSrc src;
+    typename std::conditional<X3, GemmSrcX3, GemmSrc>::type src;
     auto point_at = [&](int tile) {
         const int tile_n = tile % tiles_n, tile_m = tile / tiles_n;
         const float* Ug = U + (size_t)wino_plane_freq(pl, tile_m) * wt_gs;
-        src = gemm_src<BN>(lds, V, tile_m * BM, K, Ug, tile_n * BN, K, l);
+        if constexpr (X3) src = gemm_src_x3<BN>(lds, V, tile_m * BM, K, Ug, tile_n * BN, (int)(wt_gs * 2 / 3 / K), chunks, l);
+        else src = gemm_src<BN>(lds, V, tile_m * BM, K, Ug, tile_n * BN, K, l);
     };
+    auto load_chunk = [&](int buf) { if constexpr (X3) gemm_load_chunk_x3<BN>(src, buf); else gemm_load_chunk<BN>(src, buf); };
     using Store = GemmStore<TN, 1>;
     static_assert(Store::BYTES <= BUF * sizeof(v4f), "store scratch must fit ONE tile buffer");
     int base = 0;
     int vb = blockIdx.x;
     point_at(tile_of(vb));
-    gemm_load_chunk<BN>(src, 0);
+    load_chunk(0);
     __syncthreads();
     for (;;) {
         const int tile = tile_of(vb);
@@ -258,13 +278,16 @@
         for (int j = 0; j < TN; ++j)
 #pragma unroll
             for (int e = 0; e < 16; ++e) acc[j][e] = 0.f;
-        for (int kc = 0; kc < chunks; ++kc) gemm_chunk_f32<BN>(acc, lds, (base + kc) & 1, kc + 1 < chunks, src, l);
+        for (int kc = 0; kc < chunks; ++kc) {
+            if constexpr (X3) gemm_chunk_x3<BN>(acc, lds, (base + kc) & 1, kc + 1 < chunks, src, l);
+            else gemm_chunk_f32<BN>(acc, lds, (base + kc) & 1, kc + 1 < chunks, src, l);
+        }
         const int last = (base + chunks - 1) & 1;
         const int nvb = vb + gridDim.x;
         const bool more = nvb < ntiles;
         if (more) {
             point_at(tile_of(nvb));
-            gemm_load_chunk<BN>(src, last ^ 1);
+            load_chunk(last ^ 1);
 #if defined(__HIP_DEVICE_COMPILE__)
             __builtin_amdgcn_sched_barrier(0);
 #endif
@@ -305,6 +328,30 @@
         gemm_mma_bf16x2<TN>(acc, lds[buf], l);
         __syncthreads();
     }
+    static_assert(GemmStore<TN, JB>::BYTES <= sizeof(lds), "store scratch");
+    gemm_store_lines<TN, JB>(acc, reinterpret_cast<float*>(&lds[0][0]), M, N, m0, n0, l.wid, l.lane);
+}
+
+template <int BN, int OCC>
+__global__ __launch_bounds__(256, OCC) void wino_gemm_x3_kernel(const float* __restrict__ V, const float* __restrict__ U, float* __restrict__ M,
+                                                               const int K, const int N, const WinoPlanes pl, const long wt_gs,
+                                                               const int tiles_n, const int chunks) {
+    constexpr int BM = GEMM_BM, TN = BN / 32, JB = TN >= 2 ? 2 : 1;
+    __shared__ v4f lds[2][gemm_buf_slots_x3<BN>()];
+    const GemmLane l = gemm_lane();
+    const int tile = xcd_tile(blockIdx.x, gridDim.x);
+    const int tile_n = tile % tiles_n, tile_m = tile / tiles_n;
+    const int m0 = tile_m * BM, n0 = tile_n * BN;
+    const float* Ug = U + (size_t)wino_plane_freq(pl, tile_m) * wt_gs;
+    GemmSrcX3 src = gemm_src_x3<BN>(lds, V, m0, K, Ug, n0, (int)(wt_gs * 2 / 3 / K), chunks, l);
+    v16f acc[TN];
+#pragma unroll
+    for (int j = 0; j < TN; ++j)
+#pragma unroll
+        for (int e = 0; e < 16; ++e) acc[j][e] = 0.f;
+    gemm_load_chunk_x3<BN>(src, 0);
+    __syncthreads();
+    for (int kc = 0; kc < chunks; ++kc) gemm_chunk_x3<BN>(acc, lds, kc & 1, kc + 1 < chunks, src, l);
     static_assert(GemmStore<TN, JB>::BYTES <= sizeof(lds), "store scratch");
     gemm_store_lines<TN, JB>(acc, reinterpret_cast<float*>(&lds[0][0]), M, N, m0, n0, l.wid, l.lane);
 }
@@ -391,7 +438,23 @@
     return true;
 }
 
-void launch_wino_gemm(const ConvArgs& a, const float* wt36, const float* V, float* M, int cfg, bool bf16x2, hipStream_t s, const WinoPlanes* mix) {
+bool wino_x3_default() {
+    static const int v = [] { const char* e = getenv("FACEHIP_WINO_X3"); return e ? atoi(e) : 1; }();
+    return v != 0;
+}
+static bool wino_x3_pick_bn128(long row_tiles, int Cout, int cus) {
+    static const int force = [] { const char* e = getenv("FACEHIP_WINO_X3_BN"); return e ? atoi(e) : 0; }();
+    if (Cout % 128) return false;
+    if (force) return force == 128;
+    return row_tiles * (Cout / 128) >= wino_slots(2, cus);
+}
+bool wino_x3_pays(long row_tiles, int Cin, int Cout) {
+    (void)row_tiles; (void)Cin; (void)Cout;
+    return true;
+}
+
+void launch_wino_gemm(const ConvArgs& a, const float* wt36, const float* V, float* M, int cfg, int prec, hipStream_t s, const WinoPlanes* mix) {
+    const bool bf16x2 = prec == 1, x3 = prec == 2;
     const int TY = (a.H + 3) / 4, TX = (a.W + 3) / 4;
     const long NT = (long)a.B * TY * TX;
     if (NT <= 0) return;
@@ -429,7 +492,15 @@
             return true;
         };
         timer.begin(s);
-        if (bf16x2) {
+        if (x3) {
+            if (!wino_gemm_ok_bf16x2(a.Cin, a.Cout)) throw std::runtime_error("winograd: this layer has no three-piece bf16 GEMM");
+            g.wt_gs = (long)wino_x3_floats(conv_wt_rows(a.Cout), a.Cin);
+            if (wino_x3_pick_bn128(row_tiles, a.Cout, a.cus)) {
+                if (!launch_pers(wino_gemm_pers_kernel<128, 2, true>, 128, 2)) launch(wino_gemm_x3_kernel<128, 2>, 128);
+            } else {
+                if (!launch_pers(wino_gemm_pers_kernel<64, 2, true>, 64, 2)) launch(wino_gemm_x3_kernel<64, 2>, 64);
+            }
+        } else if (bf16x2) {
             if (!wino_gemm_ok_bf16x2(a.Cin, a.Cout)) throw std::runtime_error("winograd: this layer has no split-bf16 GEMM");
             launch(wino_gemm_bf16x2_kernel<64, 3>, 64);
         } else if (wide && a.Cout % 128 == 0 && wino_pick_bn128(row_tiles, a.Cout, mix != nullptr, a.cus)) {
@@ -450,7 +521,7 @@
             launch(wino_gemm_kernel<32, 4>, 32);
         timer.end(s, 7, g.t_flops, g.t_bytes);
     } else {
-        if (bf16x2) throw std::runtime_error("winograd: this layer has no split-bf16 GEMM");
+        if (bf16x2 || x3) throw std::runtime_error("winograd: this layer has no split-bf16 GEMM");
         launch_conv(g, cfg, s);
     }
 }
@@ -595,16 +666,17 @@
 }
 
 void launch_conv_winograd(const ConvArgs& a, const float* wt36, float* V, float* M, int cfg, const float* in_scale, const float* in_shift,
-                          hipStream_t s, bool bf16x2) {
+                          hipStream_t s, int prec) {
+    const bool bf16x2 = prec == 1;
     WinoPlanes pl;
     if (cfg == 2 && wino_mix_layout(a.B, a.H, a.W, a.Cin, a.Cout, &pl)) {
         launch_wino_mix(a, pl, nullptr, V, 0, in_scale, in_shift, bf16x2, s);
-        launch_wino_gemm(a, wt36, V, M, cfg, bf16x2, s, &pl);
+        launch_wino_gemm(a, wt36, V, M, cfg, prec, s, &pl);
         launch_wino_mix(a, pl, M, nullptr, 0, nullptr, nullptr, false, s);
         return;
     }
     launch_wino_input(a, V, in_scale, in_shift, bf16x2, s);
-    launch_wino_gemm(a, wt36, V, M, cfg, bf16x2, s);
+    launch_wino_gemm(a, wt36, V, M, cfg, prec, s);
     launch_wino_output(a, M, s);
 }
 
diff --git a/include/facehip.h b/include/facehip.h
--- a/include/facehip.h
+++ b/include/facehip.h
@@ -268,9 +268,11 @@
 FH_API int fh_rec_set_winograd(fh_rec* r, int on);
 FH_API int fh_rec_set_wino_fusion(fh_rec* r, int on);
 FH_API int fh_rec_set_shortcut_fold(fh_rec* r, int on);
-enum fh_precision { FH_PREC_FP32 = 0, FH_PREC_BF16X2 = 1 };
+enum fh_precision { FH_PREC_FP32 = 0, FH_PREC_BF16X2 = 1, FH_PREC_F32X3 = 2 };
 FH_API int fh_rec_set_precision(fh_rec* r, int mode, float* worst);
 FH_API int fh_rec_get_precision(fh_rec* r);
+FH_API int fh_rec_set_wino_x3(fh_rec* r, int on);
+FH_API int fh_rec_get_wino_x3(fh_rec* r);
 FH_API int fh_det_set_cus(fh_det* d, int cus);
 FH_API int fh_rec_set_cus(fh_rec* r, int cus);
 FH_API int fh_det_set_fused_stem(fh_det* d, int on);
```

Result: faster. 13250 faces/s, median of 6 (+5.9%).
